# hits-mbm-dev/grappa

Measured on AMD Instinct MI355X. Metric: molecules/sec (train step, energy+force loss), higher is better.
Workload: dtype f32

## Files before the change

### grappa_amd/_lib.py

```python
import ctypes as C
import os

_HERE = os.path.dirname(os.path.abspath(__file__))
LIB_PATH = os.environ.get("GRAPPA_HIP_LIB") or os.path.join(_HERE, "libgrappa_hip.so")

ABI_VERSION = 11
GEMM_GROUP4_MAX = 4
GEMM_GROUP_MAX = 16
GEMM_PRECISIONS = {"f32": 0, "f32_bf16x9": 1, "f32_bf16x6": 2, "bf16x3": 3, "bf16": 4, "f32_f16x3": 5}

c_float_p = C.POINTER(C.c_float)
c_int_p = C.POINTER(C.c_int)


class GemmDesc(C.Structure):
    _fields_ = [("M", C.c_int), ("N", C.c_int), ("K", C.c_int), ("a_kcontig", C.c_int), ("b_kcontig", C.c_int),
                ("A", C.c_void_p), ("lda", C.c_int), ("B", C.c_void_p), ("ldb", C.c_int), ("C", C.c_void_p), ("ldc", C.c_int),
                ("C2", C.c_void_p), ("ldc2", C.c_int), ("bias", C.c_void_p), ("res", C.c_void_p), ("ldres", C.c_int),
                ("aux", C.c_void_p), ("ldaux", C.c_int), ("pre", C.c_void_p), ("ldpre", C.c_int), ("a_colsum", C.c_void_p), ("act", C.c_int), ("drop_p", C.c_float), ("drop_seed", C.c_uint64),
                ("accumulate", C.c_int), ("precision", C.c_int),
                ("a_planes", C.c_int), ("b_planes", C.c_int), ("a_plane_stride", C.c_size_t), ("b_plane_stride", C.c_size_t),
                ("Cp", C.c_void_p), ("ldcp", C.c_int), ("cp_plane_stride", C.c_size_t),
                ("resp", C.c_void_p), ("ldresp", C.c_int), ("resp_plane_stride", C.c_size_t),
                ("auxp", C.c_void_p), ("ldauxp", C.c_int), ("auxp_plane_stride", C.c_size_t),
# ... 74 lines not shown
                ("n1_gamma", C.c_void_p), ("n1_beta", C.c_void_p), ("nf_gamma", C.c_void_p), ("nf_beta", C.c_void_p),
                ("drop_p", C.c_float), ("seed1", C.c_uint64), ("seed2", C.c_uint64), ("drop_salt", C.c_void_p),
                ("save_mean1", C.c_void_p), ("save_rstd1", C.c_void_p), ("save_meanf", C.c_void_p), ("save_rstdf", C.c_void_p),
                ("save_x1", C.c_void_p), ("save_qkv", C.c_void_p), ("save_att", C.c_void_p), ("save_x2", C.c_void_p), ("save_x3", C.c_void_p),
                ("save_u", C.c_void_p), ("gather_idx", C.c_void_p), ("x1_tab", C.c_void_p), ("qkv_tab", C.c_void_p), ("x2_tiled", C.c_int)]


class WriterLayerBwdDesc(C.Structure):
    _fields_ = [("s", C.c_int), ("T", C.c_int), ("F", C.c_int), ("nheads", C.c_int), ("dtype", C.c_int), ("dout", C.c_void_p),
                ("x", C.c_void_p), ("qkv", C.c_void_p), ("x2", C.c_void_p), ("u", C.c_void_p),
                ("mean1", C.c_void_p), ("rstd1", C.c_void_p), ("meanf", C.c_void_p), ("rstdf", C.c_void_p),
                ("n1_gamma", C.c_void_p), ("nf_gamma", C.c_void_p),
                ("w_in_tpk", C.c_void_p), ("w_o_tpk", C.c_void_p), ("w1_tpk", C.c_void_p), ("w2_tpk", C.c_void_p),
                ("drop_p", C.c_float), ("seed1", C.c_uint64), ("seed2", C.c_uint64), ("drop_salt", C.c_void_p),
                ("dx", C.c_void_p), ("dz2", C.c_void_p), ("dz1", C.c_void_p), ("dzo", C.c_void_p), ("dqkv", C.c_void_p),
                ("ln1_part", C.c_void_p), ("lnf_part", C.c_void_p), ("x2_tiled", C.c_int), ("gather_idx", C.c_void_p)]


WRITER_BF16 = 1

EVAL_NMOM = 10
EVAL_METRICS = ("std_energies", "std_gradients", "rmse_energies", "mae_energies", "rmse_gradients", "crmse_gradients", "mae_gradients")

COLLATE_MODES = {"copy": 0, "add": 1, "inv_rows": 2, "inc_code": 3, "conf": 4}

VP4 = C.c_void_p * 4
VP6 = C.c_void_p * 6

_vp, _i, _f, _sz, _u64 = C.c_void_p, C.c_int, C.c_float, C.c_size_t, C.c_uint64
SIGNATURES = {
    "grappa_abi_version": (_i, []),
    "grappa_build_arch": (C.c_char_p, []),
    "grappa_launch_count": (C.c_longlong, [_i]),
    "grappa_adam_step_dyn_f32": (_i, [_vp, _sz, _vp, _vp, _vp, _vp, _vp, _f, _f, _f, _f, _vp, _f, _vp, _f]),
    "grappa_split_planes_f32": (_i, [_vp, _i, _i, _vp, _i, _vp, _i, _sz, _i]),
    "grappa_split_pairs_f32": (_i, [_vp, _i, _i, _vp, _i, _vp, _vp, _i, _i]),
    "grappa_split_pairs_f32_batched": (_i, [_vp, _i, _i, _vp]),
    "grappa_amax_f32_workspace_bytes": (_sz, [_i, _i]),
    "grappa_amax_f32": (_i, [_vp, _i, _i, _vp, _i, _vp, _vp, _vp, _sz]),
    "grappa_amax_f32_batched": (_i, [_vp, _i, _vp]),
    "grappa_amax_reduce": (_i, [_vp, _i, C.POINTER(C.c_void_p), C.POINTER(C.c_int), _vp]),
    "grappa_amax_combine": (_i, [_vp, _i, _i, _vp, _vp]),
    "grappa_gemm_f32_workspace_bytes": (_sz, [_i, _i, _i]),
    "grappa_gemm_f32_plan": (_i, [_i, _i, _i, _i, c_int_p, c_int_p, c_int_p, c_int_p, c_int_p]),
    "grappa_gemm_f32_plan_desc": (_i, [C.POINTER(GemmDesc), c_int_p, c_int_p, c_int_p, c_int_p, c_int_p]),
    "grappa_gemm_f32_workspace_bytes_desc": (_sz, [C.POINTER(GemmDesc)]),
    "grappa_gemm_f32": (_i, [_vp, C.POINTER(GemmDesc), _vp, _sz]),
    "grappa_gemm_f32_grouped_workspace_bytes": (_sz, [C.POINTER(GemmDesc), _i]),
    "grappa_gemm_f32_grouped": (_i, [_vp, C.POINTER(GemmDesc), _i, _vp, _sz]),
    "grappa_gemm_f32_group_workspace_bytes": (_sz, [C.POINTER(GemmDesc), _i]),
    "grappa_gemm_f32_group": (_i, [_vp, C.POINTER(GemmDesc), _i, _vp, _sz]),
    "grappa_colsum_workspace_bytes": (_sz, [_i, _i]),
    "grappa_colsum_f32": (_i, [_vp, _i, _i, _vp, _i, _vp, _i, _vp, _sz]),
    "grappa_act_dropout_bwd_f32": (_i, [_vp, _i, _i, _vp, _i, _vp, _i, _f, _u64, _vp, _i, _vp]),
    "grappa_act_dropout_bwd_amax_f32": (_i, [_vp, _i, _i, _vp, _i, _vp, _i, _f, _u64, _vp, _i, _vp, _vp]),
    "grappa_layernorm_fwd_batched_f32": (_i, [_vp, C.POINTER(LnFwdItem), _i]),
    "grappa_layernorm_bwd_batched_f32": (_i, [_vp, C.POINTER(LnBwdItem), _i]),
    "grappa_act_dropout_bwd_batched_f32": (_i, [_vp, C.POINTER(ActDropoutItem), _i]),
    "grappa_seqattn_fwd_batched_f32": (_i, [_vp, C.POINTER(SeqAttnItem), _i]),
    "grappa_seqattn_bwd_batched_f32": (_i, [_vp, C.POINTER(SeqAttnItem), _i]),
    "grappa_act_dropout_bwd_pairs_f32": (_i, [_vp, _i, _i, _vp, _i, _vp, _i, _f, _u64, _vp, _i, _vp, _vp, _i, _vp]),
    "grappa_add_f32": (_i, [_vp, _sz, _vp, _vp, _vp]),
    "grappa_layernorm_fwd_f32": (_i, [_vp, _i, _i, _vp, _i, _vp, _vp, _vp, _i, _vp, _vp]),
    "grappa_layernorm_fwd_pairs_f32": (_i, [_vp, _i, _i, _vp, _i, _vp, _vp, _vp, _i, _vp, _vp, _vp, _vp, _i]),
    "grappa_layernorm_fwd_amax_f32": (_i, [_vp, _i, _i, _vp, _i, _vp, _vp, _vp, _i, _vp, _vp, _vp]),
    "grappa_layernorm_bwd_workspace_bytes": (_sz, [_i, _i]),
    "grappa_layernorm_bwd_partial_rows": (_i, [_i]),
    "grappa_colsum_partials_batched": (_i, [_vp, C.POINTER(ColsumItem), _i]),
    "grappa_layernorm_bwd_f32": (_i, [_vp, _i, _i, _vp, _i, _vp, _i, _vp, _vp, _vp, _vp, _i, _vp, _vp, _i, _vp, _sz]),
    "grappa_layernorm_bwd_amax_f32": (_i, [_vp, _i, _i, _vp, _i, _vp, _i, _vp, _vp, _vp, _vp, _i, _vp, _vp, _i, _vp, _sz, _vp]),
    "grappa_layernorm_bwd_drop_f32": (_i, [_vp, _i, _i, _vp, _i, _vp, _i, _vp, _vp, _vp, _vp, _i, _vp, _vp, _i, _vp, _sz, _vp, _f, _u64, _vp, _i, _vp, _vp]),
    "grappa_gat_fwd_f32": (_i, [_vp, _i, _i, _i, _i, _vp, _vp, _vp, _vp, _vp]),
    "grappa_gat_bwd_f32": (_i, [_vp, _i, _i, _i, _i, _vp, _vp, _vp, _vp, _vp, _vp, _vp, _vp, _vp]),
    "grappa_neighbor_mean_f32": (_i, [_vp, _i, _i, _vp, _vp, _vp, _vp, _i]),
    "grappa_neighbor_mean_bf16": (_i, [_vp, _i, _i, _vp, _vp, _vp, _vp, _i, _i]),
    "grappa_charge_encoding_f32": (_i, [_vp, _i, _vp, _i, _f, _f, _vp, _i, _i]),
    "grappa_tuple_gather_fwd_f32": (_i, [_vp, _i, _i, _i, _vp, _i, _vp, _vp, _vp, _i]),
    "grappa_tuple_gather_bwd_f32": (_i, [_vp, _i, _i, _vp, _vp, _vp, _i, _vp, _i, _i, _i]),
    "grappa_seqattn_fwd_f32": (_i, [_vp, _i, _i, _i, _i, _vp, _vp]),
    "grappa_seqattn_fwd_pairs_f32": (_i, [_vp, _i, _i, _i, _i, _vp, _vp, _i, _vp]),
    "grappa_seqattn_bwd_f32": (_i, [_vp, _i, _i, _i, _i, _vp, _vp, _vp]),
    "grappa_seqattn_fwd_amax_f32": (_i, [_vp, _i, _i, _i, _i, _vp, _vp, _vp]),
    "grappa_seqattn_bwd_amax_f32": (_i, [_vp, _i, _i, _i, _i, _vp, _vp, _vp, _vp]),
    "grappa_perm_concat_fwd_f32": (_i, [_vp, _i, _i, _i, _i, c_int_p, _vp, _vp]),
    "grappa_perm_concat_bwd_f32": (_i, [_vp, _i, _i, _i, _i, c_int_p, _vp, _vp]),
    "grappa_param_out_fwd_f32": (_i, [_vp, _i, _i, _i, _i, _i, _f, _vp, _i, _vp, _vp, _vp]),
    "grappa_param_out_bwd_f32": (_i, [_vp, _i, _i, _i, _i, _i, _f, _vp, _i, _vp, _vp, _vp, _vp]),
    "grappa_param_out_stats_workspace_bytes": (_sz, [_i]),
    "grappa_param_out_bwd_stats_f32": (_i, [_vp, _i, _i, _i, _i, _i, _f, _vp, _i, _vp, _vp, _vp, _vp, _vp, _sz]),
    "grappa_mm_energy_fwd_f32": (_i, [_vp, C.POINTER(MMDesc), _vp, _vp, C.POINTER(VP4), C.POINTER(VP4)]),
    "grappa_mm_gradient_fwd_f32": (_i, [_vp, C.POINTER(MMDesc), _vp]),
    "grappa_mm_bwd_f32": (_i, [_vp, C.POINTER(MMDesc), _vp, _vp, C.POINTER(VP4), C.POINTER(VP4)]),
    "grappa_nonbonded_iblock": (_i, []),
    "grappa_nonbonded_workspace_bytes": (_sz, [_i, _i, _i]),
    "grappa_nonbonded_fwd_f32": (_i, [_vp, C.POINTER(NbDesc), _vp, _vp, _vp, _vp, _sz]),
    "grappa_nonbonded_plan": (C.c_longlong, [_i, _i, _i, _vp, _vp, C.c_longlong]),
    "grappa_nonbonded_fwd_planned_f32": (_i, [_vp, C.POINTER(NbDesc), _vp, _i, _i, _vp, _vp, _vp, _vp, _sz]),
    "grappa_relax_max_atoms": (_i, []),
    "grappa_relax_fire_f32": (_i, [_vp, C.POINTER(MMDesc), C.POINTER(NbDesc), C.POINTER(RelaxOpts), _vp, _vp, _vp, _vp, _vp, _vp, _vp]),
    "grappa_relax_steps_workspace_bytes": (_sz, [_i, _i, _i, _i]),
    "grappa_relax_steps_init_f32": (_i, [_vp, C.POINTER(MMDesc), C.POINTER(NbDesc), C.POINTER(RelaxOpts), _vp, _i, _i, _vp, _sz, _vp]),
    "grappa_relax_steps_run_f32": (_i, [_vp, C.POINTER(MMDesc), C.POINTER(NbDesc), C.POINTER(RelaxOpts), _vp, _i, _i, _vp, _sz, _i, _vp]),
    "grappa_relax_steps_finish_f32": (_i, [_vp, C.POINTER(MMDesc), C.POINTER(NbDesc), C.POINTER(RelaxOpts), _vp, _i, _i, _vp, _sz,
                                           _vp, _vp, _vp, _vp, _vp, _vp, _vp]),
    "grappa_md_langevin_f32": (_i, [_vp, C.POINTER(MMDesc), C.POINTER(NbDesc), C.POINTER(MdOpts), _vp, _vp, _vp, _vp, _vp, _vp, _vp, _vp, _vp,
                                    _vp, _vp, _vp]),
    "grappa_md_philox": (None, [_u64, C.c_uint, C.c_uint, C.c_uint, C.c_uint, C.POINTER(C.c_uint * 4)]),
    "grappa_md_noise_f32": (_i, [_vp, _vp, _vp, _i, _i, _i, C.c_uint, C.c_uint, _vp]),
    "grappa_loss_ef_fwd_bwd_f32": (_i, [_vp, _i, _i, _i, _vp, _vp, _vp, _vp, _vp, _vp, _f, _f, _f, _vp, _vp, _vp]),
    "grappa_loss_param_fwd_bwd_f32": (_i, [_vp, C.POINTER(PLossDesc), _vp, C.POINTER(VP6)]),
    "grappa_eval_se_f32": (_i, [_vp, _i, _i, _i, _vp, _vp, _vp, _vp, _vp, _vp, _vp]),
    "grappa_eval_moments_f32": (_i, [_vp, _i, _i, _i, _vp, _vp, _vp, _vp, _vp, _vp, _vp]),
    "grappa_eval_bootstrap_f64": (_i, [_vp, _vp, _i, _i, _vp, _vp, _i, _i, _i, _vp, _vp, _vp]),
    "grappa_collate_batch": (_i, [_vp, _vp, C.POINTER(CollateDesc), _i, _i]),
    "grappa_sumsq_workspace_bytes": (_sz, [_sz]),
    "grappa_sumsq_f32": (_i, [_vp, _sz, _vp, _vp, _i, _vp, _sz]),
    "grappa_adam_step_f32": (_i, [_vp, _sz, _vp, _vp, _vp, _vp, _f, _f, _f, _f, _f, _i, _f, _vp, _f]),
    "grappa_dropout_keep": (_i, [_u64, _u64, _f]),
    "grappa_layernorm_fwd_bf16": (_i, [_vp, _i, _i, _vp, _i, _vp, _vp, _vp, _i, _vp, _vp]),
    "grappa_layernorm_bwd_bf16": (_i, [_vp, _i, _i, _vp, _i, _vp, _i, _vp, _vp, _vp, _vp, _i, _vp, _vp, _i, _vp, _sz]),
    "grappa_act_dropout_bwd_bf16": (_i, [_vp, _i, _i, _vp, _i, _vp, _i, _f, _u64, _vp, _i, _vp]),
    "grappa_gat_fwd_bf16": (_i, [_vp, _i, _i, _i, _i, _vp, _vp, _vp, _vp, _vp]),
    "grappa_gat_bwd_bf16": (_i, [_vp, _i, _i, _i, _i, _vp, _vp, _vp, _vp, _vp, _vp, _vp, _vp, _vp]),
    "grappa_tuple_gather_fwd_bf16": (_i, [_vp, _i, _i, _i, _vp, _i, _vp, _vp, _vp, _i]),
    "grappa_tuple_gather_bwd_bf16": (_i, [_vp, _i, _i, _vp, _vp, _vp, _i, _vp, _i, _i, _i]),
    "grappa_seqattn_fwd_bf16": (_i, [_vp, _i, _i, _i, _i, _vp, _vp]),
    "grappa_seqattn_bwd_bf16": (_i, [_vp, _i, _i, _i, _i, _vp, _vp, _vp]),
    "grappa_perm_concat_fwd_bf16": (_i, [_vp, _i, _i, _i, _i, c_int_p, _vp, _vp]),
    "grappa_perm_concat_bwd_bf16": (_i, [_vp, _i, _i, _i, _i, c_int_p, _vp, _vp]),
    "grappa_convert_f32_to_bf16": (_i, [_vp, _i, _i, _vp, _i, _vp, _i]),
    "grappa_convert_bf16_to_f32": (_i, [_vp, _i, _i, _vp, _i, _vp, _i]),
    "grappa_writer_head_fwd": (_i, [_vp, C.POINTER(WriterLayerDesc)]),
    "grappa_writer_head_bwd": (_i, [_vp, C.POINTER(WriterLayerBwdDesc)]),
    "grappa_writer_head_tiles": (_i, [_i, _i]),
    "grappa_writer_pack_bytes": (_sz, [_i, _i, _i]),
    "grappa_writer_pack_weight": (_i, [_vp, _i, _i, _vp, _i, _i, _i, _vp]),
}

_lib = None


def load():
    global _lib
    if _lib is not None:
        return _lib
    if not os.path.exists(LIB_PATH):
        raise RuntimeError(f"{LIB_PATH} is missing: build it with `python -c 'import __graft_entry__ as g; g.build()'` "
                           f"or `make -C grappa_amd/csrc` (there is no CPU fallback for the Grappa HIP path)")
    lib = C.CDLL(LIB_PATH)
    for name, (res, args) in SIGNATURES.items():
        fn = getattr(lib, name)
        fn.restype = res
        fn.argtypes = args
    if lib.grappa_abi_version() != ABI_VERSION:
        raise RuntimeError("libgrappa_hip.so: ABI version mismatch")
    _lib = lib
    return lib


def nonbonded_iblock() -> int:
    return int(load().grappa_nonbonded_iblock())


def relax_max_atoms() -> int:
    return int(load().grappa_relax_max_atoms())

# ... 6 lines not shown
```

### grappa_amd/backend.py

```python
from __future__ import annotations

import ctypes as C
import os
import weakref
from collections import namedtuple
from typing import List, NamedTuple, Optional, Sequence

import torch

from . import _lib
from ._marshal import GrappaHipError, _chk, _flat, _ptr
from .backend_mm import MMBackend

_BACKEND = None


def set_backend(b) -> None:
    global _BACKEND
    _BACKEND = b


def get_backend():
    global _BACKEND
    if _BACKEND is None:
# ... 64 lines not shown
    precision: int

    @property
    def fmt(self) -> str:
        return self.name if self.name in ("pairs", "wpairs") else ("planes" if self.name.endswith("planes") else "f32")

    @property
    def fp16_split(self) -> bool:
        return self.name in ("pairs", "wpairs", "split")


class _PendingGemm:
    __slots__ = ("d", "route", "shape", "flops", "nbytes", "ret", "dev", "keep", "groupable", "key")

    def __init__(self, d, route, shape, flops, nbytes, ret, dev, keep, groupable):
        self.d, self.route, self.shape, self.flops, self.nbytes, self.ret, self.dev, self.keep, self.groupable = d, route, shape, flops, nbytes, ret, dev, keep, groupable
        self.key = (route.name, route.name == "split" and route.layout, route.precision)


_PlanesEntry = namedtuple("_PlanesEntry", "ver planes ref")
_PairsTable = namedtuple("_PairsTable", "tab n tiles keep")
_AmaxTable = namedtuple("_AmaxTable", "tab n")
_PairsRefresh = namedtuple("_PairsRefresh", "event captured ordered")
_WgradItem = namedtuple("_WgradItem", "dz x dw db am pz px")
_LnItem = namedtuple("_LnItem", "part nrows W dgamma_ptr dbeta_ptr dgamma dbeta stream task")


class _PairsEntry:
    __slots__ = ("ver", "pairs", "ref", "epoch", "transposed", "amax")

    def __init__(self, ver, pairs, ref, epoch, transposed, amax):
        self.ver, self.pairs, self.ref, self.epoch, self.transposed, self.amax = ver, pairs, ref, epoch, transposed, amax


class _AmaxEntry:
    __slots__ = ("ver", "w", "amax", "epoch", "batchable")

    def __init__(self, ver, w, amax, epoch, batchable):
        self.ver, self.w, self.amax, self.epoch, self.batchable = ver, w, amax, epoch, batchable


class HipBackend(MMBackend):
    name = "hip"

    def __init__(self):
        if not torch.cuda.is_available():
            raise RuntimeError("grappa_amd needs an AMD GPU (torch.cuda.is_available() is False); there is no CPU fallback")
        self.lib = _lib.load()
        self._ws = {}
        self._ws_need = {}
        self.set_gemm_precision(os.environ.get("GRAPPA_GEMM_PRECISION", DEFAULT_GEMM_PRECISION))
        self.set_gemm_precision_bwd(os.environ.get("GRAPPA_GEMM_PRECISION_BWD") or None)
        self._prof = None
        self.defer_wgrads = os.environ.get("GRAPPA_DEFER_WGRADS", "1") not in ("0", "")
        self._wq = {}
        self.defer_ln = os.environ.get("GRAPPA_DEFER_LN_REDUCTIONS", "1") not in ("0", "")
        self._lnq = []
        self._tasks = set()
        self.wgrad_queue_bytes = int(float(os.environ.get("GRAPPA_WGRAD_QUEUE_GB", "12")) * 2 ** 30)
        self.inference_pairs = os.environ.get("GRAPPA_INFERENCE_PAIRS", "1") not in ("0", "")
        self.training_pairs = os.environ.get("GRAPPA_TRAINING_PAIRS", "1") not in ("0", "")
        self.group_launches = os.environ.get("GRAPPA_GROUP_LAUNCHES", "1") not in ("0", "")
        self.amax_parts = os.environ.get("GRAPPA_AMAX_PARTS", "0") not in ("0", "")
        self.fuse_ln_drop = os.environ.get("GRAPPA_FUSE_LN_DROP", "1") not in ("0", "")
        self.pairs_min_rows = int(os.environ.get("GRAPPA_PAIRS_MIN_ROWS", "12288"))
        self.backward_pairs = os.environ.get("GRAPPA_BACKWARD_PAIRS", "0") not in ("0", "")
        self.weight_pairs_min_rows = int(os.environ.get("GRAPPA_WPAIRS_MIN_ROWS", "24000"))
        self._tails = None
        self._salt = None
        self._salt_ptr = None
        self.plan_override = None
        self.splitk_reduce = 0
        self._tails_pinned = False
        if os.environ.get("GRAPPA_PLAN_TAILS", "") != "":
            self.pin_tail_launches(os.environ["GRAPPA_PLAN_TAILS"] != "0")
        self.gnn_tails = os.environ.get("GRAPPA_GNN_TAILS", "0") not in ("0", "")
        self.wgrads_aside = os.environ.get("GRAPPA_WGRADS_ASIDE", "1") not in ("0", "")
        self._side_streams = {}
        self._aside = []
        self.weight_planes = os.environ.get("GRAPPA_WEIGHT_PLANES", "0") not in ("0", "")
        self.fused_writer_layer = os.environ.get("GRAPPA_FUSED_WRITER_LAYER", "1") not in ("0", "")
        self.fused_writer_layer_bwd = os.environ.get("GRAPPA_FUSED_WRITER_LAYER_BWD", "1") not in ("0", "")
        self.fused_first_layer = os.environ.get("GRAPPA_FUSED_FIRST_LAYER", "1") not in ("0", "")
        self._wplanes = {}
        self._wpairs = {}
        self._wptable = None
        self._wpairs_ready = None
        self._wepoch = 0
        self._wamax = {}
        self._wtable = None
        self.wgrad_column_maxima = os.environ.get("GRAPPA_WGRAD_COLUMN_MAXIMA", "0") not in ("0", "")

    def set_gemm_precision(self, name: str) -> None:
        if name not in _lib.GEMM_PRECISIONS:
            raise ValueError(f"gemm precision {name!r}: expected one of {sorted(_lib.GEMM_PRECISIONS)}")
        self.gemm_precision_name = name
        self.gemm_precision = _lib.GEMM_PRECISIONS[name]

    def set_gemm_precision_bwd(self, name) -> None:
        if name is not None and name not in _lib.GEMM_PRECISIONS:
            raise ValueError(f"gemm precision {name!r}: expected one of {sorted(_lib.GEMM_PRECISIONS)}")
        self.gemm_precision_bwd_name = name
        self.gemm_precision_bwd = None if name is None else _lib.GEMM_PRECISIONS[name]

    def invalidate_weight_planes(self) -> None:
        self._wepoch += 1

    def invalidate_weights(self) -> None:
        self._wepoch += 1

    def _cached_form(self, w: torch.Tensor, tag, alloc, fill) -> torch.Tensor:
        key = (w.data_ptr(), *w.shape, tag)
        ver = (w._version, self._wepoch)
        hit = self._wplanes.get(key)
        if hit is not None and hit.ref() is not w:
            hit = None
        if hit is not None and hit.ver == ver:
            return hit.planes
        if hit is not None:
            t = hit.planes
        else:
            t = alloc()
            for k in [k for k, e in self._wplanes.items() if e.ref() is None]:
                del self._wplanes[k]
        fill(t)
        self._wplanes[key] = _PlanesEntry(ver, t, weakref.ref(w))
        return t

    def _planes_of_weight(self, w: torch.Tensor, transposed: bool) -> torch.Tensor:
        R, Cc = w.shape
        rows, cols = (Cc, R) if transposed else (R, Cc)
        return self._cached_form(
            w, transposed, lambda: torch.zeros((3, (rows + 31) // 32 * 32, (cols + 31) // 32 * 32), dtype=torch.bfloat16, device=w.device),
            lambda pl: _chk(self.lib.grappa_split_planes_f32(self._stream(), R, Cc, w.data_ptr(), _f32_2d(w, "W", w.device), pl.data_ptr(), pl.stride(1),
                                                             pl.stride(0), int(transposed)), "grappa_split_planes_f32"))

    def _pairs_of_weight(self, w: torch.Tensor, transposed: bool = False) -> torch.Tensor:
        R, Cc = w.shape
        key = (w.data_ptr(), R, Cc, "pairsT" if transposed else "pairs")
        ver = (w._version, self._wepoch)
        hit = self._wpairs.get(key)
        if hit is not None and hit.ref() is not w:
            hit = None
        if hit is not None:
            hit.epoch = self._wepoch
            if hit.ver == ver:
                self._after_pairs_refresh()
                return hit.pairs
            self._refresh_weight_pairs()
            if hit.ver == ver:
                return hit.pairs
        am = self._amax_of_weight(w)
        rows, cols = (Cc, R) if transposed else (R, Cc)
        pairs = torch.zeros((rows, 2 * ((cols + 31) // 32 * 32)), dtype=torch.float16, device=w.device)
        _chk(self.lib.grappa_split_pairs_f32(self._stream(), R, Cc, w.data_ptr(), _f32_2d(w, "W", w.device), (am.col if transposed else am.row).data_ptr(),
                                             pairs.data_ptr(), pairs.stride(0), int(transposed)), "grappa_split_pairs_f32")
        for k in [k for k, e in self._wpairs.items() if e.ref() is None]:
            del self._wpairs[k]
        self._wpairs[key] = _PairsEntry(ver, pairs, weakref.ref(w), self._wepoch, transposed, am)
        self._wptable = None
        return pairs

    def _refresh_weight_pairs(self) -> None:
        import numpy as np
        ageing = not torch.cuda.is_current_stream_capturing()
        for k in [k for k, e in self._wpairs.items() if e.ref() is None or (ageing and e.epoch < self._wepoch - 1)]:
# ... 958 lines not shown
    def _csr_check(self, plan, N, dev):
        if plan.N != N or plan.indptr.device != dev or plan.indptr.dtype != torch.int32 or plan.indptr.numel() != N + 1:
            raise ValueError("graph plan does not match the feature tensor (atoms / device)")
        if plan.indices.numel() != plan.E or plan.rev.numel() != plan.E:
            raise ValueError("graph plan: edge arrays")

    def gat_fwd(self, plan, ft, H, D, out, alpha) -> None:
        dev = out.device
        N = ft.shape[0]
        self._csr_check(plan, N, dev)
        dt = _same_dtype(ft, out)
        _flat(ft, "ft", dev, dt), _flat(out, "out", dev, dt), _flat(alpha, "alpha", dev)
        if ft.shape[1] != H * D or out.shape != ft.shape or alpha.numel() != plan.E * H:
            raise ValueError("gat_fwd: shapes")
        eb = ft.element_size()
        nbytes = plan.E * (H * D * eb + 4) + N * (2 * H * D * eb + 4)
        fn = getattr(self.lib, f"grappa_gat_fwd_{_sfx(ft)}")
        self._timed("gat_fwd", 2.0 * plan.E * H * D * 2, nbytes,
                    lambda: _chk(fn(self._stream(), N, plan.E, H, D, plan.indptr.data_ptr(), plan.indices.data_ptr(),
                                    ft.data_ptr(), out.data_ptr(), alpha.data_ptr()), "grappa_gat_fwd"))

    def gat_bwd(self, plan, ft, out, alpha, dout, H, D, dft) -> None:
        dev = dft.device
        N = ft.shape[0]
        self._csr_check(plan, N, dev)
        dt = _same_dtype(ft, out, dout, dft)
        for t, n in ((ft, "ft"), (out, "out"), (dout, "dout"), (dft, "dft")):
            _flat(t, n, dev, dt)
        _flat(alpha, "alpha", dev)
        if ft.shape[1] != H * D or out.shape != ft.shape or dout.shape != ft.shape or dft.shape != ft.shape or alpha.numel() != plan.E * H:
            raise ValueError("gat_bwd: shapes")
        delta = torch.empty((N, H), dtype=torch.float32, device=dev)
        eb = ft.element_size()
        nbytes = plan.E * (2 * H * D * eb + 4) + N * (4 * H * D * eb + 4)
        fn = getattr(self.lib, f"grappa_gat_bwd_{_sfx(ft)}")
        self._timed("gat_bwd", 2.0 * plan.E * H * D * 5, nbytes,
                    lambda: _chk(fn(self._stream(), N, plan.E, H, D, plan.indptr.data_ptr(), plan.indices.data_ptr(),
                                    plan.rev.data_ptr(), ft.data_ptr(), out.data_ptr(), alpha.data_ptr(), dout.data_ptr(),
                                    dft.data_ptr(), delta.data_ptr()), "grappa_gat_bwd"))

    def neighbor_mean(self, plan, x, out, scale_by_neighbor: bool) -> None:
        dev = out.device
        N, F = x.shape
        self._csr_check(plan, N, dev)
        if out.shape != x.shape:
            raise ValueError("neighbor_mean: shapes")
        if x.dtype == torch.bfloat16:
            _flat(x, "x", dev, torch.bfloat16), _flat(out, "out", dev, out.dtype)
            if out.dtype not in _ACT_DTYPES:
                raise ValueError("neighbor_mean: out must be bfloat16 or float32")
            _chk(self.lib.grappa_neighbor_mean_bf16(self._stream(), N, F, plan.indptr.data_ptr(), plan.indices.data_ptr(), x.data_ptr(), out.data_ptr(),
                                                    int(out.dtype == torch.float32), int(scale_by_neighbor)), "grappa_neighbor_mean_bf16")
            return
        _flat(x, "x", dev), _flat(out, "out", dev)
        _chk(self.lib.grappa_neighbor_mean_f32(self._stream(), N, F, plan.indptr.data_ptr(), plan.indices.data_ptr(), x.data_ptr(), out.data_ptr(),
                                               int(scale_by_neighbor)), "grappa_neighbor_mean_f32")

    def charge_encoding(self, q, dim, lo, hi, out, col0) -> None:
        dev = out.device
        _flat(q, "q", dev)
        N = q.numel()
        if out.shape[0] != N or col0 + dim > out.shape[1]:
            raise ValueError("charge_encoding: shapes")
        _chk(self.lib.grappa_charge_encoding_f32(self._stream(), N, q.data_ptr(), dim, float(lo), float(hi), out.data_ptr(), _f32_2d(out, "out", dev),
                                                 col0), "grappa_charge_encoding_f32")

    def tuple_gather_fwd(self, a, idx, s, pe, x) -> None:
        dev = x.device
        T = idx.shape[0]
        W = x.shape[1]
        if idx.dtype != torch.int32 or idx.device != dev or not idx.is_contiguous() or (T and idx.shape[1] != s):
            raise ValueError("tuple_gather_fwd: idx must be contiguous int32 (T,s)")
        if x.shape[0] != s * T or a.shape[1] < W:
            raise ValueError("tuple_gather_fwd: shapes")
        if pe is not None:
            _flat(pe, "pe", dev)
            if pe.numel() != s:
                raise ValueError("tuple_gather_fwd: pe length")
        dt = _same_dtype(a, x)
        fn = getattr(self.lib, f"grappa_tuple_gather_fwd_{_sfx(x)}")
        _chk(fn(self._stream(), T, s, W, a.data_ptr(), _f32_2d(a, "a", dev, dt), idx.data_ptr(), _ptr(pe),
                x.data_ptr(), _f32_2d(x, "x", dev, dt)), "grappa_tuple_gather_fwd")

    def tuple_gather_bwd(self, inv_ptr, inv_rows, dx, da, has_pe: bool, accumulate=False) -> None:
        dev = da.device
        N, W = da.shape[0], dx.shape[1]
        if inv_ptr.dtype != torch.int32 or inv_ptr.numel() != N + 1 or inv_ptr.device != dev or inv_rows.dtype != torch.int32:
            raise ValueError("tuple_gather_bwd: inverse incidence")
        if da.shape[1] < W or inv_rows.numel() != dx.shape[0]:
            raise ValueError("tuple_gather_bwd: shapes")
        dt = _same_dtype(dx, da)
        fn = getattr(self.lib, f"grappa_tuple_gather_bwd_{_sfx(da)}")
        _chk(fn(self._stream(), N, W, inv_ptr.data_ptr(), inv_rows.data_ptr(), dx.data_ptr(),
                _f32_2d(dx, "dx", dev, dt), da.data_ptr(), _f32_2d(da, "da", dev, dt), int(has_pe), int(accumulate)),
             "grappa_tuple_gather_bwd")

    def seqattn_fwd(self, qkv, s, T, nheads, out, amax=None, pairs=False):
        if pairs:
            dev = qkv.device
            F = qkv.shape[1] // 3
            if qkv.dtype != torch.float32 or qkv.shape != (s * T, 3 * F) or F % nheads or F % 32 or F > 512:
                raise ValueError("seqattn_fwd: the pair format needs float32 q, k, v of F % 32 == 0, F <= 512 columns each")
            _flat(qkv, "qkv", dev)
            row = torch.empty(s * T, dtype=torch.int32, device=dev)
            pr = torch.empty((s * T, 2 * F), dtype=torch.float16, device=dev)
            if T:
                _chk(self.lib.grappa_seqattn_fwd_pairs_f32(self._stream(), s, T, nheads, F // nheads, qkv.data_ptr(), pr.data_ptr(), pr.stride(0),
                                                           row.data_ptr()), "grappa_seqattn_fwd_pairs_f32")
            return Amax(row=row, pairs=pr)
        dev = out.device
        dt = _same_dtype(qkv, out)
        _flat(qkv, "qkv", dev, dt), _flat(out, "out", dev, dt)
        F = out.shape[1]
        if qkv.shape != (s * T, 3 * F) or out.shape[0] != s * T or F % nheads:
            raise ValueError("seqattn_fwd: shapes")
        row = self._new_row_amax(out, False, amax)
        args = (self._stream(), s, T, nheads, F // nheads, qkv.data_ptr(), out.data_ptr())
        if row is not None:
            _chk(self.lib.grappa_seqattn_fwd_amax_f32(*args, row.data_ptr()), "grappa_seqattn_fwd_amax_f32")
            return Amax(row=row)
        _chk(getattr(self.lib, f"grappa_seqattn_fwd_{_sfx(out)}")(*args), "grappa_seqattn_fwd")
        return None

    def _packed_weight(self, w: torch.Tensor, transposed: bool = False) -> torch.Tensor:
        R, Cc = w.shape
        N, K = (Cc, R) if transposed else (R, Cc)
        return self._cached_form(
            w, "packT" if transposed else "pack", lambda: torch.empty(N * K, dtype=torch.bfloat16, device=w.device),
            lambda pk: _chk(self.lib.grappa_writer_pack_weight(self._stream(), N, K, w.data_ptr(), _f32_2d(w, "W", w.device), int(transposed), _lib.WRITER_BF16,
                                                               pk.data_ptr()), "grappa_writer_pack_weight"))

    def writer_layer_ok(self, x: torch.Tensor, s: int, nheads: int, *params) -> bool:
        if not self.fused_writer_layer or x.dtype != torch.bfloat16 or x.dim() != 2 or x.shape[1] != 512 or nheads != 8 or s not in (2, 3, 4):
            return False
        if x.shape[0] == 0:
            return False
        return all(p is not None and p.dtype == torch.float32 and p.is_contiguous() for p in params)

    def writer_layer_fwd(self, x, s, T, nheads, drop_p, seed1, seed2, n1_w, n1_b, w_in, b_in, w_o, b_o, nf_w, nf_b, w1, b1, w2, b2, out, save=None, gather=None):
        dev = out.device
        M, Fd = out.shape
        d = _lib.WriterLayerDesc()
        d.s, d.T, d.F, d.nheads, d.dtype = s, T, Fd, nheads, _lib.WRITER_BF16
        _flat(out, "out", dev, torch.bfloat16)
        d.out = out.data_ptr()
        if gather is not None:
            idx_tab, x1_tab, qkv_tab = gather
            if M != s * T or idx_tab.dtype != torch.int32 or tuple(idx_tab.shape) != (T, s) or not idx_tab.is_contiguous() or idx_tab.device != dev:
                raise ValueError("writer_layer_fwd: gather index")
            _flat(x1_tab, "x1_tab", dev, torch.bfloat16), _flat(qkv_tab, "qkv_tab", dev, torch.bfloat16)
            if x1_tab.shape[1] != Fd or tuple(qkv_tab.shape) != (x1_tab.shape[0], 3 * Fd):
                raise ValueError("writer_layer_fwd: gather tables")
            d.gather_idx, d.x1_tab, d.qkv_tab = idx_tab.data_ptr(), x1_tab.data_ptr(), qkv_tab.data_ptr()
        else:
            if tuple(x.shape) != (M, Fd) or M != s * T or out.dtype != x.dtype:
                raise ValueError("writer_layer_fwd: shapes")
            _flat(x, "x", dev, torch.bfloat16)
            d.x = x.data_ptr()
        for name, wt, shape in (("w_in_pk", w_in, (3 * Fd, Fd)), ("w_o_pk", w_o, (Fd, Fd)), ("w1_pk", w1, (Fd, Fd)), ("w2_pk", w2, (Fd, Fd))):
            if gather is not None and name == "w_in_pk":
                continue
            if tuple(wt.shape) != shape:
                raise ValueError(f"writer_layer_fwd: {name[:-3]} has shape {tuple(wt.shape)}, expected {shape}")
            setattr(d, name, self._packed_weight(wt).data_ptr())
        for name, v, n in (("b_in", b_in, 3 * Fd), ("b_o", b_o, Fd), ("b1", b1, Fd), ("b2", b2, Fd), ("n1_gamma", n1_w, Fd), ("n1_beta", n1_b, Fd),
                           ("nf_gamma", nf_w, Fd), ("nf_beta", nf_b, Fd)):
            if gather is not None and name.startswith("n1_"):
                continue
            _flat(v, name, dev)
            if v.numel() != n:
                raise ValueError(f"writer_layer_fwd: {name} length")
            setattr(d, name, v.data_ptr())
        d.drop_p, d.seed1, d.seed2 = float(drop_p), int(seed1) & (2 ** 64 - 1), int(seed2) & (2 ** 64 - 1)
        d.drop_salt = self._salt_ptr
        keep = None
        if save is not None:
            for name in ("meanf", "rstdf") if gather is not None else ("mean1", "rstd1", "meanf", "rstdf"):
                t = save[name]
                _flat(t, name, dev)
                if t.numel() != M:
                    raise ValueError(f"writer_layer_fwd: save[{name!r}] length")
                setattr(d, "save_" + name, t.data_ptr())
            tiles = self.lib.grappa_writer_head_tiles(s, T)
            d.x2_tiled = int(bool(save.get("x2_tiled", False)))
            for name in ("att", "x2", "x3", "u") if gather is not None else ("x1", "qkv", "att", "x2", "x3", "u"):
                t = save[name]
                _flat(t, name, dev, torch.bfloat16)
                want = (tiles * 64, Fd) if (name == "x2" and d.x2_tiled) else (M, 3 * Fd if name == "qkv" else Fd)
                if tuple(t.shape) != want:
                    raise ValueError(f"writer_layer_fwd: save[{name!r}] shape {tuple(t.shape)}, expected {want}")
                setattr(d, "save_" + name, t.data_ptr())
            keep = save
        nprod = 3 if gather is not None else 6
        flops = 2.0 * M * Fd * (nprod * Fd) + 4.0 * M * s * Fd
        nbytes = 2.0 * M * Fd * ((5 if gather is not None else 2) + ((5 if gather is not None else 9) if save is not None else 0)) + 2.0 * nprod * Fd * Fd
        self._timed("writer_layer", flops, nbytes, lambda: _chk(self.lib.grappa_writer_head_fwd(self._stream(), C.byref(d)), "grappa_writer_head_fwd"),
                    lambda: [{"M": M, "s": s, "save": keep is not None, "gather": gather is not None}])

    def writer_layer_bwd(self, dout, x, s, T, nheads, drop_p, seed1, seed2, saved, n1_w, n1_b, w_in, w_o, nf_w, nf_b, w1, w2, gather=None):
        dev = dout.device
        M, Fd = dout.shape
        bf = torch.bfloat16
        if M != s * T:
            raise ValueError("writer_layer_bwd: shapes")
        d = _lib.WriterLayerBwdDesc()
        d.s, d.T, d.F, d.nheads, d.dtype = s, T, Fd, nheads, _lib.WRITER_BF16
        ntiles = self.lib.grappa_writer_head_tiles(s, T)
        d.x2_tiled = int(bool(saved.get("x2_tiled", False)))
        if gather is not None:
            idx_tab, qkv_tab = gather
            if idx_tab.dtype != torch.int32 or tuple(idx_tab.shape) != (T, s) or not idx_tab.is_contiguous() or qkv_tab.shape[1] != 3 * Fd:
                raise ValueError("writer_layer_bwd: gather arguments")
            d.gather_idx = idx_tab.data_ptr()
            tensors = (("dout", dout, (M, Fd)), ("qkv", qkv_tab, tuple(qkv_tab.shape)), ("x2", saved["x2"], (ntiles * 64, Fd) if d.x2_tiled else (M, Fd)),
                       ("u", saved["u"], (M, Fd)))
        else:
            tensors = (("dout", dout, (M, Fd)), ("x", x, (M, Fd)), ("qkv", saved["qkv"], (M, 3 * Fd)),
                       ("x2", saved["x2"], (ntiles * 64, Fd) if d.x2_tiled else (M, Fd)), ("u", saved["u"], (M, Fd)))
        for name, t, shape in tensors:
            _flat(t, name, dev, bf)
            if tuple(t.shape) != shape:
                raise ValueError(f"writer_layer_bwd: {name} shape")
            setattr(d, name, t.data_ptr())
        for name in ("meanf", "rstdf") if gather is not None else ("mean1", "rstd1", "meanf", "rstdf"):
            _flat(saved[name], name, dev)
            setattr(d, name, saved[name].data_ptr())
        _flat(nf_w, "nf_gamma", dev)
        d.nf_gamma = nf_w.data_ptr()
        if gather is None:
            _flat(n1_w, "n1_gamma", dev)
            d.n1_gamma = n1_w.data_ptr()
        for name, wt in (("w_in_tpk", w_in), ("w_o_tpk", w_o), ("w1_tpk", w1), ("w2_tpk", w2)):
            if gather is not None and name == "w_in_tpk":
                continue
            setattr(d, name, self._packed_weight(wt, transposed=True).data_ptr())
        d.drop_p, d.seed1, d.seed2, d.drop_salt = float(drop_p), int(seed1) & (2 ** 64 - 1), int(seed2) & (2 ** 64 - 1), self._salt_ptr
        new = lambda *sh: torch.empty(sh, dtype=bf, device=dev)
        dx, dz2, dz1, dzo, dqkv = new(M, Fd), new(M, Fd), new(M, Fd), new(M, Fd), new(M, 3 * Fd)
        parts = torch.empty((2, ntiles, 2, Fd), dtype=torch.float32, device=dev)
        d.dx, d.dz2, d.dz1, d.dzo, d.dqkv = dx.data_ptr(), dz2.data_ptr(), dz1.data_ptr(), dzo.data_ptr(), dqkv.data_ptr()
        d.ln1_part, d.lnf_part = parts[0].data_ptr(), parts[1].data_ptr()
        nprod = 3 if gather is not None else 6
        flops = 2.0 * M * Fd * (nprod * Fd) + 8.0 * M * s * Fd
        self._timed("writer_layer", flops, 2.0 * M * Fd * 15 + 2.0 * nprod * Fd * Fd,
                    lambda: _chk(self.lib.grappa_writer_head_bwd(self._stream(), C.byref(d)), "grappa_writer_head_bwd"),
                    lambda: [{"M": M, "s": s, "bwd": True, "gather": gather is not None}])
        for part, g, b in ((parts[1], nf_w, nf_b),) if gather is not None else ((parts[0], n1_w, n1_b), (parts[1], nf_w, nf_b)):
            self._reduce_ln_partials(part, ntiles, Fd, g, b)
        return dx, dz2, dz1, dzo, dqkv

    def _reduce_ln_partials(self, part, nrows, W, gamma, beta) -> None:
        from .ops import _pgrad
        dg = _pgrad(gamma) if gamma.requires_grad else torch.zeros_like(gamma)
        db = _pgrad(beta) if beta.requires_grad else torch.zeros_like(beta)
        task = self._queue_flush() if (self.defer_wgrads and self.defer_ln) else -1
        if task >= 0 and all(q.dgamma_ptr != dg.data_ptr() for q in self._lnq if q.task == task):
            self._lnq.append(_LnItem(part, nrows, W, dg.data_ptr(), db.data_ptr(), dg, db, torch.cuda.current_stream(), task))
            return
        arr = (_lib.ColsumItem * 1)()
        a = arr[0]
        a.part, a.nrows, a.n, a.out, a.out2, a.n_first, a.accumulate = part.data_ptr(), nrows, 2 * W, dg.data_ptr(), db.data_ptr(), W, 1
        _chk(self.lib.grappa_colsum_partials_batched(self._stream(), arr, 1), "grappa_colsum_partials_batched")

    def seqattn_bwd(self, qkv, dout, s, T, nheads, dqkv, amax=None):
        dev = dqkv.device
        dt = _same_dtype(qkv, dout, dqkv)
        _flat(qkv, "qkv", dev, dt), _flat(dout, "dout", dev, dt), _flat(dqkv, "dqkv", dev, dt)
        F = dout.shape[1]
        if qkv.shape != (s * T, 3 * F) or dqkv.shape != qkv.shape or dout.shape[0] != s * T:
            raise ValueError("seqattn_bwd: shapes")
        row = self._new_row_amax(dqkv, True, amax)
        args = (self._stream(), s, T, nheads, F // nheads, qkv.data_ptr(), dout.data_ptr(), dqkv.data_ptr())
        if row is not None:
            _chk(self.lib.grappa_seqattn_bwd_amax_f32(*args, row.data_ptr()), "grappa_seqattn_bwd_amax_f32")
            return Amax(row=row)
        _chk(getattr(self.lib, f"grappa_seqattn_bwd_{_sfx(dqkv)}")(*args), "grappa_seqattn_bwd")
        return None

    def perm_concat_fwd(self, x, s, T, perms: Sequence[Sequence[int]], z) -> None:
        dev = z.device
        dt = _same_dtype(x, z)
        _flat(x, "x", dev, dt), _flat(z, "z", dev, dt)
        F, P = x.shape[1], len(perms)
        if x.shape[0] != s * T or z.shape != (P * T, s * F):
            raise ValueError("perm_concat_fwd: shapes")
        arr = (C.c_int * (P * s))(*[int(v) for p in perms for v in p])
        fn = getattr(self.lib, f"grappa_perm_concat_fwd_{_sfx(z)}")
        _chk(fn(self._stream(), s, T, F, P, arr, x.data_ptr(), z.data_ptr()), "grappa_perm_concat_fwd")

    def perm_concat_bwd(self, dz, s, T, perms, dx) -> None:
        dev = dx.device
        dt = _same_dtype(dz, dx)
        _flat(dz, "dz", dev, dt), _flat(dx, "dx", dev, dt)
        F, P = dx.shape[1], len(perms)
        if dx.shape[0] != s * T or dz.shape != (P * T, s * F):
            raise ValueError("perm_concat_bwd: shapes")
        arr = (C.c_int * (P * s))(*[int(v) for p in perms for v in p])
        fn = getattr(self.lib, f"grappa_perm_concat_bwd_{_sfx(dx)}")
        _chk(fn(self._stream(), s, T, F, P, arr, dz.data_ptr(), dx.data_ptr()), "grappa_perm_concat_bwd")

    def param_out_fwd(self, kind, o, T, P, n_per, gated, cutoff, consts, k, eq) -> None:
        dev = k.device
        _flat(o, "o", dev), _flat(consts, "consts", dev), _flat(k, "k", dev)
        if o.shape[0] != P * T:
            raise ValueError("param_out_fwd: shapes")
        if eq is not None:
            _flat(eq, "eq", dev)
        _chk(self.lib.grappa_param_out_fwd_f32(self._stream(), kind, T, P, n_per, int(gated), float(cutoff), o.data_ptr(), o.shape[1],
                                               consts.data_ptr(), k.data_ptr(), _ptr(eq)), "grappa_param_out_fwd_f32")

    def param_out_bwd(self, kind, o, T, P, n_per, gated, cutoff, consts, dk, deq, d_o) -> None:
        dev = d_o.device
        _flat(o, "o", dev), _flat(consts, "consts", dev), _flat(d_o, "d_o", dev)
        for t, n in ((dk, "dk"), (deq, "deq")):
            if t is not None:
                _flat(t, n, dev)
        if o.shape[0] != P * T or d_o.shape != o.shape:
            raise ValueError("param_out_bwd: shapes")
        _chk(self.lib.grappa_param_out_bwd_f32(self._stream(), kind, T, P, n_per, int(gated), float(cutoff), o.data_ptr(), o.shape[1],
                                               consts.data_ptr(), _ptr(dk), _ptr(deq), d_o.data_ptr()), "grappa_param_out_bwd_f32")

    def param_out_bwd_stats(self, kind, o, T, P, n_per, gated, cutoff, consts, dk, deq, d_consts) -> None:
        dev = d_consts.device
        _flat(o, "o", dev), _flat(consts, "consts", dev), _flat(d_consts, "d_consts", dev)
        if o.shape[0] != P * T or d_consts.numel() != consts.numel():
            raise ValueError("param_out_bwd_stats: shapes")
        ws = self._workspace(self.lib.grappa_param_out_stats_workspace_bytes(T), dev)
        _chk(self.lib.grappa_param_out_bwd_stats_f32(self._stream(), kind, T, P, n_per, int(gated), float(cutoff), _ptr(o), o.shape[1] if o.dim() == 2 else 0,
                                                     consts.data_ptr(), _ptr(dk), _ptr(deq), d_consts.data_ptr(), ws.data_ptr(), ws.numel()),
             "grappa_param_out_bwd_stats_f32")

    def loss_ef(self, plan, energy, energy_ref, is_dummy, grad, grad_ref, wE, wG, inv_B, loss_mol, gE, gG) -> None:
        dev = loss_mol.device
        B = _loss_mols(plan)
        Cc = energy.shape[1] if energy is not None else grad.shape[1]
        for t, n in ((energy, "energy"), (energy_ref, "energy_ref"), (is_dummy, "is_dummy"), (grad, "grad"), (grad_ref, "grad_ref"),
                     (gE, "gE"), (gG, "gG"), (loss_mol, "loss_mol")):
            if t is not None:
                _flat(t, n, dev)
        _chk(self.lib.grappa_loss_ef_fwd_bwd_f32(self._stream(), B, Cc, plan.N, plan.atom_molptr.data_ptr(), _ptr(energy), _ptr(energy_ref),
                                                 _ptr(is_dummy), _ptr(grad), _ptr(grad_ref), float(wE), float(wG), float(inv_B),
                                                 loss_mol.data_ptr(), _ptr(gE), _ptr(gG)), "grappa_loss_ef_fwd_bwd_f32")

    def collate_gather(self, tables, B: int) -> None:
        if not tables or B == 0:
            return
        dev = tables[0]["dst"].device
        arr = (_lib.CollateDesc * len(tables))()
        for d, t in zip(arr, tables):
            for k in ("src", "dst"):
                if t[k].element_size() not in (4, 8) or t[k].device != dev or not t[k].is_contiguous():
                    raise ValueError(f"collate table {k}: expected a contiguous 4- or 8-byte tensor on {dev}")
            for k, dt in (("src_row", torch.int64), ("dst_row", torch.int64), ("p0", torch.int32), ("p1", torch.int32)):
                v = t.get(k)
# ... 130 lines not shown
```

### grappa_amd/capture.py

```python
from __future__ import annotations

from typing import Callable, Dict, Optional, Tuple

import torch

from .backend import get_backend


def _pinned_by_graph(be):
    return (list(be._wamax.values()), be._wtable, list(be._wpairs.values()), be._wptable, dict(be._wplanes), dict(be._ws), getattr(be, "_salt", None),
            dict(be._side_streams))


def _touch_weight_caches(be) -> None:
    for e in be._wamax.values():
        e.epoch = be._wepoch
    for e in be._wpairs.values():
        e.epoch = be._wepoch


def _drop_outputs(g) -> None:
    for lvl in ("n2", "n3", "n4", "n4_improper"):
        for k in ("k", "eq"):
            g.nodes[lvl].data.pop(k, None)
# ... 186 lines not shown
        self.plan = g.plan()
        for lvl in ("n2", "n3", "n4", "n4_improper"):
            if self.plan.T[lvl]:
                self.plan.position_tables(lvl)
        self.signature = train_signature(g)
        self._rehome_inputs()
        self.stream = torch.cuda.Stream(device=g.device)
        self.stream.wait_stream(torch.cuda.current_stream(g.device))
        with torch.cuda.stream(self.stream), torch.no_grad():
            for _ in range(max(int(warmup), 3)):
                self.be.invalidate_weights()
                self._eager()
        self.stream.synchronize()
        self.be.invalidate_weights()
        self.graph = torch.cuda.CUDAGraph()
        with torch.cuda.graph(self.graph, stream=self.stream), torch.no_grad():
            self._eager()
        self._pinned = _pinned_by_graph(self.be)
        torch.cuda.current_stream(g.device).wait_stream(self.stream)

    def _eager(self):
        _drop_outputs(self.g)
        return self.energy(self.model(self.g))

    def __call__(self):
        self.graph.replay()
        _touch_weight_caches(self.be)
        return self.g


def train_signature(g) -> tuple:
    plan = g.plan()
    return (tuple(int(g.num_nodes(nt)) for nt in ("n1", "n2", "n3", "n4", "n4_improper", "g")), int(g.num_edges()), getattr(plan, "n_real_mols", None),
            tuple(sorted((nt, k, tuple(v.shape), str(v.dtype)) for nt, d in g._data.items() for k, v in d.items() if torch.is_tensor(v))))


class CapturedForward:

    def __init__(self, model, g, warmup: int = 2, refresh_weights: bool = False):
        self.model, self.g = model, g
        self.refresh_weights = bool(refresh_weights)
        self.be = get_backend()
        self.plan = g.plan()
        for lvl in ("n2", "n3", "n4", "n4_improper"):
            if self.plan.T[lvl]:
                self.plan.position_tables(lvl)
        self._rehome_inputs()
        self.stream = torch.cuda.Stream(device=g.device)
        self.stream.wait_stream(torch.cuda.current_stream(g.device))
        with torch.cuda.stream(self.stream), torch.no_grad():
            for _ in range(max(int(warmup), 3 if self.refresh_weights else 1)):
                if self.refresh_weights:
                    self.be.invalidate_weights()
                _drop_outputs(g)
                model(g)
        self.stream.synchronize()
        if self.refresh_weights:
            self.be.invalidate_weights()
        self.weights_stamp = self._stamp()
        self.config_stamp = self._config_stamp()
        self.graph = torch.cuda.CUDAGraph()
        with torch.cuda.graph(self.graph, stream=self.stream), torch.no_grad():
            _drop_outputs(g)
            model(g)
            self.outputs: Dict[Tuple[str, str], torch.Tensor] = {(lvl, k): g.nodes[lvl].data[k] for lvl in ("n2", "n3", "n4", "n4_improper")
                                                                for k in ("k", "eq") if k in g.nodes[lvl].data}
            self.out_flat = torch.cat([t.reshape(-1).float() for t in self.outputs.values()]) if self.outputs else None
        self._pinned = _pinned_by_graph(self.be)
        torch.cuda.current_stream(g.device).wait_stream(self.stream)
        self.out_host = torch.empty(self.out_flat.shape, dtype=torch.float32).pin_memory() if self.out_flat is not None else None

    def _stamp(self):
        ps = self.__dict__.get("_params")
        if ps is None:
            ps = self._params = list(self.model.parameters())
        return (self.be._wepoch, sum(p._version for p in ps))

    def _config_stamp(self):
        be = self.be
        ps = self.__dict__.get("_params")
        if ps is None:
            ps = self._params = list(self.model.parameters())
        return (be.gemm_precision_name, getattr(be, "gemm_precision_bwd", None), be.inference_pairs, be.training_pairs, be._tails, be.plan_override,
                be.splitk_reduce, be.weight_pairs_min_rows, be.pairs_min_rows, tuple(p.data_ptr() for p in ps))

    def valid(self) -> bool:
        if self._config_stamp() != self.config_stamp:
            return False
        return self.refresh_weights or self._stamp() == self.weights_stamp

    def replay(self):
        self.graph.replay()
        if self.refresh_weights:
            _touch_weight_caches(self.be)
        return self.g

    @staticmethod
    def signature(g) -> tuple:
        return (tuple(int(g.num_nodes(nt)) for nt in ("n1", "n2", "n3", "n4", "n4_improper", "g")), int(g.num_edges()),
                tuple(sorted((k, tuple(v.shape), str(v.dtype)) for k, v in g._data["n1"].items() if torch.is_tensor(v) and k != "h")))

    @staticmethod
    def _plan_tensors(plan):
        out = {}
        for name, val in vars(plan).items():
            if torch.is_tensor(val):
                out[name] = val
            elif isinstance(val, dict):
                for k, v in val.items():
                    if torch.is_tensor(v):
                        out[f"{name}.{k}"] = v
                    elif isinstance(v, tuple):
                        for i, t in enumerate(v):
                            if torch.is_tensor(t):
                                out[f"{name}.{k}.{i}"] = t
        return out

    def _input_slots(self, plan, g):
        slots = dict(self._plan_tensors(plan))
        for k, t in g._data["n1"].items():
            if torch.is_tensor(t) and k != "h":
                slots["n1." + k] = t
        return slots

    def _rehome_inputs(self) -> None:
        slots = self._input_slots(self.plan, self.g)
        self._layout, off = {}, 0
        for name, t in slots.items():
            nbytes = t.numel() * t.element_size()
            self._layout[name] = (off, nbytes, t.dtype, tuple(t.shape))
            off += (nbytes + 15) // 16 * 16
        self._in_dev = torch.zeros(max(off, 16), dtype=torch.uint8, device=self.g.device)
        self._in_host = torch.zeros(max(off, 16), dtype=torch.uint8).pin_memory()
        self._host_views = {name: self._in_host[o:o + nbytes].view(dtype).view(shape) for name, (o, nbytes, dtype, shape) in self._layout.items()}
        views = {}
        for name, (o, nbytes, dtype, shape) in self._layout.items():
            v = self._in_dev[o:o + nbytes].view(dtype).view(shape)
            v.copy_(slots[name])
            views[name] = v
        for name, v in views.items():
            parts = name.split(".")
            if parts[0] == "n1":
                self.g._data["n1"][name[3:]] = v
            elif len(parts) == 1:
                setattr(self.plan, name, v)
            elif len(parts) == 2:
                getattr(self.plan, parts[0])[parts[1]] = v
            else:
                d = getattr(self.plan, parts[0])
                tup = list(d[parts[1]])
                tup[int(parts[2])] = v
                d[parts[1]] = tuple(tup)

    def load(self, g_host) -> None:
        plan = g_host.plan()
        for lvl in self.plan.__dict__.get("_pos_tables", {}):
            plan.position_tables(lvl)
        src = self._input_slots(plan, g_host)
        if set(src) != set(self._layout):
            raise ValueError("load: the graph has other input tables than the captured one")
        for name, (o, nbytes, dtype, shape) in self._layout.items():
            t = src[name]
            if tuple(t.shape) != shape or t.dtype != dtype:
                raise ValueError(f"load: {name} is {t.dtype} {tuple(t.shape)}, the captured graph holds {dtype} {shape}")
            self._host_views[name].copy_(t)
        self._in_dev.copy_(self._in_host, non_blocking=True)

# ... 49 lines not shown
```

### grappa_amd/csrc/tuples.hip

```cpp
#include "common.h"

namespace {

struct Perms {
    int p[6][4];
};

template <typename TA, typename TX>
__global__ __launch_bounds__(256) void tuple_gather_fwd_kernel(int T, int s, int W, const TA* __restrict__ a, int lda,
                                                               const int* __restrict__ idx, const float* __restrict__ pe,
                                                               TX* __restrict__ x, int ldx) {
    const int lane = threadIdx.x & 63;
    const int nrows = s * T, nvec = W >> 2;
    const int wave0 = (blockIdx.x * blockDim.x + threadIdx.x) >> 6, nw = (gridDim.x * blockDim.x) >> 6;
    for (int r = wave0; r < nrows; r += nw) {
        const int pos = r / T, t = r - pos * T;
        const int atom = idx[(size_t)t * s + pos];
        const TA* src = a + (size_t)atom * lda;
        TX* dst = x + (size_t)r * ldx;
        const float pev = pe ? pe[pos] : 0.f;
        for (int c = lane; c < nvec; c += 64) {
            float4 v = ld4(src, c);
            if (pe && c == nvec - 1) v.w = pev;
            st4(dst, c, v);
        }
    }
}

template <typename TX, typename TA>
__global__ __launch_bounds__(256) void tuple_gather_bwd_kernel(int N, int W, const int* __restrict__ inv_ptr, const int* __restrict__ inv_rows,
                                                               const TX* __restrict__ dx, int lddx, TA* __restrict__ da, int ldda,
                                                               int has_pe, int accumulate) {
    const int lane = threadIdx.x & 63;
    const int nvec = W >> 2;
    const int n = (blockIdx.x * blockDim.x + threadIdx.x) >> 6;
    if (n >= N) return;
    const int r0 = inv_ptr[n], r1 = inv_ptr[n + 1];
    TA* dst = da + (size_t)n * ldda;
    for (int c = lane; c < nvec; c += 64) {
        float4 acc = accumulate ? ld4(dst, c) : make_float4(0.f, 0.f, 0.f, 0.f);
        for (int j = r0; j < r1; ++j) {
            float4 v = ld4(dx + (size_t)inv_rows[j] * lddx, c);
            if (has_pe && c == nvec - 1) v.w = 0.f;
            acc.x += v.x; acc.y += v.y; acc.z += v.z; acc.w += v.w;
        }
        st4(dst, c, acc);
    }
}

__device__ inline float dot4(const float4& a, const float4& b) { return (a.x * b.x + a.y * b.y) + (a.z * b.z + a.w * b.w); }

__device__ inline unsigned mag4(const float4& v) {
    return max(max(__float_as_uint(v.x) & 0x7fffffffu, __float_as_uint(v.y) & 0x7fffffffu),
               max(__float_as_uint(v.z) & 0x7fffffffu, __float_as_uint(v.w) & 0x7fffffffu));
}
__device__ inline unsigned wave_umax(unsigned v) {
#pragma unroll
    for (int o = 32; o > 0; o >>= 1) v = max(v, (unsigned)__shfl_xor((int)v, o, 64));
    return v;
}

template <int S, typename TE>
__device__ __forceinline__ void seqattn_fwd_body(int T, int F, int dh, const TE* __restrict__ qkv, TE* __restrict__ out,
                                                 unsigned* __restrict__ row_amax, int vblock) {
    const int lane = threadIdx.x & 63;
    const int t = (vblock * blockDim.x + threadIdx.x) >> 6;
    if (t >= T) return;
    const int nvec = F >> 2, lph = dh >> 2;
    const float scale = 1.0f / sqrtf((float)dh);
    unsigned am[S];
#pragma unroll
    for (int i = 0; i < S; ++i) am[i] = 0u;
    for (int c0 = 0; c0 < nvec; c0 += 64) {
        const int c = c0 + lane;
        const bool ok = c < nvec;
        float4 q[S], k[S], v[S];
#pragma unroll
        for (int i = 0; i < S; ++i) {
            const TE* row = qkv + ((size_t)i * T + t) * 3 * F;
            q[i] = ok ? ld4(row, c) : make_float4(0.f, 0.f, 0.f, 0.f);
            k[i] = ok ? ld4(row, nvec + c) : make_float4(0.f, 0.f, 0.f, 0.f);
            v[i] = ok ? ld4(row, 2 * nvec + c) : make_float4(0.f, 0.f, 0.f, 0.f);
        }
#pragma unroll
        for (int i = 0; i < S; ++i) {
            float sc[S], mx = -INFINITY;
#pragma unroll
            for (int j = 0; j < S; ++j) {
                sc[j] = group_sum(dot4(q[i], k[j]), lph) * scale;
                mx = fmaxf(mx, sc[j]);
            }
            float den = 0.f;
#pragma unroll
            for (int j = 0; j < S; ++j) {
                sc[j] = expf(sc[j] - mx);
                den += sc[j];
            }
            const float inv = 1.0f / den;
            float4 o = make_float4(0.f, 0.f, 0.f, 0.f);
#pragma unroll
            for (int j = 0; j < S; ++j) {
                const float p = sc[j] * inv;
                o.x += p * v[j].x; o.y += p * v[j].y; o.z += p * v[j].z; o.w += p * v[j].w;
            }
            if (ok) {
                st4(out + ((size_t)i * T + t) * F, c, o);
                am[i] = max(am[i], mag4(o));
            }
        }
    }
    if (row_amax) {
#pragma unroll
        for (int i = 0; i < S; ++i) {
            const unsigned m = wave_umax(am[i]);
            if (lane == 0) row_amax[(size_t)i * T + t] = m;
        }
    }
}

template <int S, typename TE>
__global__ __launch_bounds__(256) void seqattn_fwd_kernel(int T, int F, int dh, const TE* __restrict__ qkv, TE* __restrict__ out,
                                                          unsigned* __restrict__ row_amax) {
    seqattn_fwd_body<S, TE>(T, F, dh, qkv, out, row_amax, blockIdx.x);
}

struct SeqAttnBatch {
    grappa_seqattn_item it[GRAPPA_ROW_BATCH_MAX];
    int blk_begin[GRAPPA_ROW_BATCH_MAX + 1];
    int count;
};
__global__ __launch_bounds__(256) void seqattn_fwd_batched_kernel(SeqAttnBatch b) {
    int i = 0;
    while (i + 1 < b.count && (int)blockIdx.x >= b.blk_begin[i + 1]) ++i;
    const grappa_seqattn_item& t = b.it[i];
    const int vb = (int)blockIdx.x - b.blk_begin[i], F = t.nheads * t.dh;
    switch (t.s) {
        case 1: seqattn_fwd_body<1, float>(t.T, F, t.dh, t.qkv, t.out, t.amax, vb); break;
        case 2: seqattn_fwd_body<2, float>(t.T, F, t.dh, t.qkv, t.out, t.amax, vb); break;
        case 3: seqattn_fwd_body<3, float>(t.T, F, t.dh, t.qkv, t.out, t.amax, vb); break;
        default: seqattn_fwd_body<4, float>(t.T, F, t.dh, t.qkv, t.out, t.amax, vb); break;
    }
}

template <int S>
__global__ __launch_bounds__(256) void seqattn_fwd_pairs_kernel(int T, int F, int dh, const float* __restrict__ qkv, uint16_t* __restrict__ pairs, int ldp,
                                                                unsigned* __restrict__ row_amax) {
    const int lane = threadIdx.x & 63;
    const int t = (blockIdx.x * blockDim.x + threadIdx.x) >> 6;
    if (t >= T) return;
    const int nvec = F >> 2, lph = dh >> 2;
    const float scale = 1.0f / sqrtf((float)dh);
    unsigned am[S];
    float4 keep[2][S];
#pragma unroll
    for (int i = 0; i < S; ++i) am[i] = 0u;
#pragma unroll
    for (int trip = 0; trip < 2; ++trip) {
        const int c = trip * 64 + lane;
        const bool ok = c < nvec;
        float4 q[S], k[S], v[S];
#pragma unroll
        for (int i = 0; i < S; ++i) {
            const float* row = qkv + ((size_t)i * T + t) * 3 * F;
            q[i] = ok ? ld4(row, c) : make_float4(0.f, 0.f, 0.f, 0.f);
            k[i] = ok ? ld4(row, nvec + c) : make_float4(0.f, 0.f, 0.f, 0.f);
            v[i] = ok ? ld4(row, 2 * nvec + c) : make_float4(0.f, 0.f, 0.f, 0.f);
        }
#pragma unroll
        for (int i = 0; i < S; ++i) {
            float sc[S], mx = -INFINITY;
#pragma unroll
            for (int j = 0; j < S; ++j) {
                sc[j] = group_sum(dot4(q[i], k[j]), lph) * scale;
                mx = fmaxf(mx, sc[j]);
            }
            float den = 0.f;
#pragma unroll
            for (int j = 0; j < S; ++j) {
                sc[j] = expf(sc[j] - mx);
                den += sc[j];
            }
            const float inv = 1.0f / den;
            float4 o = make_float4(0.f, 0.f, 0.f, 0.f);
#pragma unroll
            for (int j = 0; j < S; ++j) {
                const float p = sc[j] * inv;
                o.x += p * v[j].x; o.y += p * v[j].y; o.z += p * v[j].z; o.w += p * v[j].w;
            }
            keep[trip][i] = o;
            if (ok) am[i] = max(am[i], mag4(o));
        }
    }
#pragma unroll
    for (int i = 0; i < S; ++i) {
        const unsigned m = wave_umax(am[i]);
        const int shift = grappa_amax_shift(m);
        uint16_t* pr = pairs + ((size_t)i * T + t) * ldp;
#pragma unroll
        for (int trip = 0; trip < 2; ++trip) {
            const int c = trip * 64 + lane;
            st_pairs4_paired(pr, c, keep[trip][i], shift, c < nvec);
        }
        if (lane == 0) row_amax[(size_t)i * T + t] = m;
    }
}

template <int S, typename TE>
__device__ __forceinline__ void seqattn_bwd_body(int T, int F, int dh, const TE* __restrict__ qkv, const TE* __restrict__ dout,
                                                 TE* __restrict__ dqkv, unsigned* __restrict__ row_amax, int vblock) {
    const int lane = threadIdx.x & 63;
    const int t = (vblock * blockDim.x + threadIdx.x) >> 6;
    if (t >= T) return;
    const int nvec = F >> 2, lph = dh >> 2;
    const float scale = 1.0f / sqrtf((float)dh);
    const float4 zero = make_float4(0.f, 0.f, 0.f, 0.f);
    unsigned am[S];
#pragma unroll
    for (int i = 0; i < S; ++i) am[i] = 0u;
    for (int c0 = 0; c0 < nvec; c0 += 64) {
        const int c = c0 + lane;
        const bool ok = c < nvec;
        float4 q[S], k[S], v[S], go[S], dq[S], dk[S], dv[S];
#pragma unroll
        for (int i = 0; i < S; ++i) {
            const TE* row = qkv + ((size_t)i * T + t) * 3 * F;
            q[i] = ok ? ld4(row, c) : zero;
            k[i] = ok ? ld4(row, nvec + c) : zero;
            v[i] = ok ? ld4(row, 2 * nvec + c) : zero;
            go[i] = ok ? ld4(dout + ((size_t)i * T + t) * F, c) : zero;
            dq[i] = zero; dk[i] = zero; dv[i] = zero;
        }
#pragma unroll
        for (int i = 0; i < S; ++i) {
            float p[S], dp[S], mx = -INFINITY;
#pragma unroll
            for (int j = 0; j < S; ++j) {
                p[j] = group_sum(dot4(q[i], k[j]), lph) * scale;
                mx = fmaxf(mx, p[j]);
            }
            float den = 0.f;
#pragma unroll
            for (int j = 0; j < S; ++j) {
                p[j] = expf(p[j] - mx);
                den += p[j];
            }
            const float inv = 1.0f / den;
            float dsum = 0.f;
#pragma unroll
            for (int j = 0; j < S; ++j) {
                p[j] *= inv;
                dp[j] = group_sum(dot4(go[i], v[j]), lph);
                dsum += p[j] * dp[j];
            }
#pragma unroll
            for (int j = 0; j < S; ++j) {
                const float ds = p[j] * (dp[j] - dsum) * scale;
                dq[i].x += ds * k[j].x; dq[i].y += ds * k[j].y; dq[i].z += ds * k[j].z; dq[i].w += ds * k[j].w;
                dk[j].x += ds * q[i].x; dk[j].y += ds * q[i].y; dk[j].z += ds * q[i].z; dk[j].w += ds * q[i].w;
                dv[j].x += p[j] * go[i].x; dv[j].y += p[j] * go[i].y; dv[j].z += p[j] * go[i].z; dv[j].w += p[j] * go[i].w;
            }
        }
        if (ok) {
#pragma unroll
            for (int i = 0; i < S; ++i) {
                TE* row = dqkv + ((size_t)i * T + t) * 3 * F;
                st4(row, c, dq[i]);
                st4(row, nvec + c, dk[i]);
                st4(row, 2 * nvec + c, dv[i]);
                am[i] = max(am[i], max(mag4(dq[i]), max(mag4(dk[i]), mag4(dv[i]))));
            }
        }
    }
    if (row_amax) {
#pragma unroll
        for (int i = 0; i < S; ++i) {
            const unsigned m = wave_umax(am[i]);
            if (lane == 0) row_amax[(size_t)i * T + t] = m;
        }
    }
}

template <int S, typename TE>
__global__ __launch_bounds__(256) void seqattn_bwd_kernel(int T, int F, int dh, const TE* __restrict__ qkv, const TE* __restrict__ dout,
                                                          TE* __restrict__ dqkv, unsigned* __restrict__ row_amax) {
    seqattn_bwd_body<S, TE>(T, F, dh, qkv, dout, dqkv, row_amax, blockIdx.x);
}

__global__ __launch_bounds__(256) void seqattn_bwd_batched_kernel(SeqAttnBatch b) {
    int i = 0;
    while (i + 1 < b.count && (int)blockIdx.x >= b.blk_begin[i + 1]) ++i;
    const grappa_seqattn_item& t = b.it[i];
    const int vb = (int)blockIdx.x - b.blk_begin[i], F = t.nheads * t.dh;
    switch (t.s) {
        case 1: seqattn_bwd_body<1, float>(t.T, F, t.dh, t.qkv, t.dout, t.dqkv, t.amax, vb); break;
        case 2: seqattn_bwd_body<2, float>(t.T, F, t.dh, t.qkv, t.dout, t.dqkv, t.amax, vb); break;
        case 3: seqattn_bwd_body<3, float>(t.T, F, t.dh, t.qkv, t.dout, t.dqkv, t.amax, vb); break;
        default: seqattn_bwd_body<4, float>(t.T, F, t.dh, t.qkv, t.dout, t.dqkv, t.amax, vb); break;
    }
}

template <int S, int E, typename TE>
__global__ __launch_bounds__(256) void seqattn_fwd_kernel_e(int T, int F, int dh, const TE* __restrict__ qkv, TE* __restrict__ out) {
    const int lane = threadIdx.x & 63;
    const int t = (blockIdx.x * blockDim.x + threadIdx.x) >> 6;
    if (t >= T) return;
    const int nvec = F / E, lph = dh / E;
    const float scale = 1.0f / sqrtf((float)dh);
    for (int c0 = 0; c0 < nvec; c0 += 64) {
        const int c = c0 + lane;
        const bool ok = c < nvec;
        Chunk<E> q[S], k[S], v[S];
#pragma unroll
        for (int i = 0; i < S; ++i) {
            const TE* row = qkv + ((size_t)i * T + t) * 3 * F;
            q[i] = ok ? ldc<E, TE>(row, c) : chunk_zero<E>();
            k[i] = ok ? ldc<E, TE>(row, nvec + c) : chunk_zero<E>();
            v[i] = ok ? ldc<E, TE>(row, 2 * nvec + c) : chunk_zero<E>();
        }
#pragma unroll
        for (int i = 0; i < S; ++i) {
            float sc[S], mx = -INFINITY;
#pragma unroll
            for (int j = 0; j < S; ++j) {
                sc[j] = group_sum(cdot<E>(q[i], k[j]), lph) * scale;
                mx = fmaxf(mx, sc[j]);
            }
            float den = 0.f;
#pragma unroll
            for (int j = 0; j < S; ++j) {
                sc[j] = expf(sc[j] - mx);
                den += sc[j];
            }
            const float inv = 1.0f / den;
            Chunk<E> o = chunk_zero<E>();
#pragma unroll
            for (int j = 0; j < S; ++j) {
                const float p = sc[j] * inv;
#pragma unroll
                for (int e = 0; e < E; ++e) o.v[e] += p * v[j].v[e];
            }
            if (ok) stc<E, TE>(out + ((size_t)i * T + t) * F, c, o);
        }
    }
}

template <int S, int E, typename TE>
__global__ __launch_bounds__(256) void seqattn_bwd_kernel_e(int T, int F, int dh, const TE* __restrict__ qkv, const TE* __restrict__ dout,
                                                            TE* __restrict__ dqkv) {
    const int lane = threadIdx.x & 63;
    const int t = (blockIdx.x * blockDim.x + threadIdx.x) >> 6;
    if (t >= T) return;
    const int nvec = F / E, lph = dh / E;
    const float scale = 1.0f / sqrtf((float)dh);
    for (int c0 = 0; c0 < nvec; c0 += 64) {
        const int c = c0 + lane;
        const bool ok = c < nvec;
        Chunk<E> q[S], k[S], v[S], go[S], dq[S], dk[S], dv[S];
#pragma unroll
        for (int i = 0; i < S; ++i) {
            const TE* row = qkv + ((size_t)i * T + t) * 3 * F;
            q[i] = ok ? ldc<E, TE>(row, c) : chunk_zero<E>();
            k[i] = ok ? ldc<E, TE>(row, nvec + c) : chunk_zero<E>();
            v[i] = ok ? ldc<E, TE>(row, 2 * nvec + c) : chunk_zero<E>();
            go[i] = ok ? ldc<E, TE>(dout + ((size_t)i * T + t) * F, c) : chunk_zero<E>();
            dq[i] = chunk_zero<E>(); dk[i] = chunk_zero<E>(); dv[i] = chunk_zero<E>();
        }
#pragma unroll
        for (int i = 0; i < S; ++i) {
// ... 303 lines not shown
    if constexpr (sizeof(TE) == 2) {
        if ((dh & 7) == 0 && pow2(dh / 8) &&
            ((reinterpret_cast<uintptr_t>(qkv) | reinterpret_cast<uintptr_t>(dout) | reinterpret_cast<uintptr_t>(dqkv)) & 15) == 0) {
            switch (s) {
                case 1: GRAPPA_LAUNCH((seqattn_bwd_kernel_e<1, 8, TE>), grid, dim3(256), 0, st, T, F, dh, qkv, dout, dqkv); break;
                case 2: GRAPPA_LAUNCH((seqattn_bwd_kernel_e<2, 8, TE>), grid, dim3(256), 0, st, T, F, dh, qkv, dout, dqkv); break;
                case 3: GRAPPA_LAUNCH((seqattn_bwd_kernel_e<3, 8, TE>), grid, dim3(256), 0, st, T, F, dh, qkv, dout, dqkv); break;
                default: GRAPPA_LAUNCH((seqattn_bwd_kernel_e<4, 8, TE>), grid, dim3(256), 0, st, T, F, dh, qkv, dout, dqkv); break;
            }
            return grappa_launch_status();
        }
    }
    switch (s) {
        case 1: GRAPPA_LAUNCH((seqattn_bwd_kernel<1, TE>), grid, dim3(256), 0, st, T, F, dh, qkv, dout, dqkv, row_amax); break;
        case 2: GRAPPA_LAUNCH((seqattn_bwd_kernel<2, TE>), grid, dim3(256), 0, st, T, F, dh, qkv, dout, dqkv, row_amax); break;
        case 3: GRAPPA_LAUNCH((seqattn_bwd_kernel<3, TE>), grid, dim3(256), 0, st, T, F, dh, qkv, dout, dqkv, row_amax); break;
        default: GRAPPA_LAUNCH((seqattn_bwd_kernel<4, TE>), grid, dim3(256), 0, st, T, F, dh, qkv, dout, dqkv, row_amax); break;
    }
    return grappa_launch_status();
}
}

extern "C" int grappa_tuple_gather_fwd_f32(void* stream, int T, int s, int W, const float* a, int lda, const int* idx, const float* pe,
                                           float* x, int ldx) {
    return tuple_gather_fwd_impl<float, float>(stream, T, s, W, a, lda, idx, pe, x, ldx);
}
extern "C" int grappa_tuple_gather_fwd_bf16(void* stream, int T, int s, int W, const uint16_t* a, int lda, const int* idx, const float* pe,
                                            uint16_t* x, int ldx) {
    return tuple_gather_fwd_impl<grappa_bf16_t, grappa_bf16_t>(stream, T, s, W, a, lda, idx, pe, x, ldx);
}
extern "C" int grappa_tuple_gather_bwd_f32(void* stream, int N, int W, const int* inv_ptr, const int* inv_rows, const float* dx, int lddx,
                                           float* da, int ldda, int has_pe, int accumulate) {
    return tuple_gather_bwd_impl<float, float>(stream, N, W, inv_ptr, inv_rows, dx, lddx, da, ldda, has_pe, accumulate);
}
extern "C" int grappa_tuple_gather_bwd_bf16(void* stream, int N, int W, const int* inv_ptr, const int* inv_rows, const uint16_t* dx, int lddx,
                                            uint16_t* da, int ldda, int has_pe, int accumulate) {
    return tuple_gather_bwd_impl<grappa_bf16_t, grappa_bf16_t>(stream, N, W, inv_ptr, inv_rows, dx, lddx, da, ldda, has_pe, accumulate);
}
namespace {
int seqattn_batch(const grappa_seqattn_item* items, int count, bool bwd, SeqAttnBatch& b) {
    if (!items || count <= 0 || count > GRAPPA_ROW_BATCH_MAX) return GRAPPA_ERR_ARG;
    b.count = count;
    b.blk_begin[0] = 0;
    for (int i = 0; i < count; ++i) {
        const grappa_seqattn_item& t = items[i];
        if (t.s < 1 || t.s > 4 || t.T < 0 || t.nheads <= 0 || t.dh <= 0 || (t.dh & 3) || !pow2(t.dh / 4) || t.dh / 4 > 64 || t.nheads * t.dh > 1024) return GRAPPA_ERR_ARG;
        if (t.T > 0) {
            if (!t.qkv || !aligned_el<float>(t.qkv)) return GRAPPA_ERR_ARG;
            if (bwd ? (!t.dout || !t.dqkv || !aligned_el<float>(t.dout) || !aligned_el<float>(t.dqkv)) : (!t.out || !aligned_el<float>(t.out))) return GRAPPA_ERR_ARG;
        }
        b.it[i] = t;
        b.blk_begin[i + 1] = b.blk_begin[i] + (t.T + 3) / 4;
    }
    for (int i = count; i < GRAPPA_ROW_BATCH_MAX; ++i) b.blk_begin[i + 1] = b.blk_begin[count];
    return GRAPPA_OK;
}
}

extern "C" int grappa_seqattn_fwd_batched_f32(void* stream, const grappa_seqattn_item* items, int count) {
    SeqAttnBatch b;
    const int rc = seqattn_batch(items, count, false, b);
    if (rc != GRAPPA_OK || b.blk_begin[count] == 0) return rc;
    GRAPPA_LAUNCH(seqattn_fwd_batched_kernel, dim3(b.blk_begin[count]), dim3(256), 0, reinterpret_cast<hipStream_t>(stream), b);
    return grappa_launch_status();
}
extern "C" int grappa_seqattn_bwd_batched_f32(void* stream, const grappa_seqattn_item* items, int count) {
    SeqAttnBatch b;
    const int rc = seqattn_batch(items, count, true, b);
    if (rc != GRAPPA_OK || b.blk_begin[count] == 0) return rc;
    GRAPPA_LAUNCH(seqattn_bwd_batched_kernel, dim3(b.blk_begin[count]), dim3(256), 0, reinterpret_cast<hipStream_t>(stream), b);
    return grappa_launch_status();
}

extern "C" int grappa_seqattn_fwd_f32(void* stream, int s, int T, int nheads, int dh, const float* qkv, float* out) {
    return seqattn_fwd_impl<float>(stream, s, T, nheads, dh, qkv, out);
}
extern "C" int grappa_seqattn_fwd_amax_f32(void* stream, int s, int T, int nheads, int dh, const float* qkv, float* out, uint32_t* out_amax) {
    return seqattn_fwd_impl<float>(stream, s, T, nheads, dh, qkv, out, out_amax);
}
extern "C" int grappa_seqattn_bwd_amax_f32(void* stream, int s, int T, int nheads, int dh, const float* qkv, const float* dout, float* dqkv,
                                           uint32_t* dqkv_amax) {
    return seqattn_bwd_impl<float>(stream, s, T, nheads, dh, qkv, dout, dqkv, dqkv_amax);
}
extern "C" int grappa_seqattn_fwd_pairs_f32(void* stream, int s, int T, int nheads, int dh, const float* qkv, uint16_t* pairs, int ldp,
                                            uint32_t* out_amax) {
    const int F = nheads * dh;
    if (s < 1 || s > 4 || T < 0 || nheads <= 0 || dh <= 0 || (dh & 3) || !pow2(dh / 4) || dh / 4 > 64 || F > 512 || (F & 31) || ldp < 2 * F || (ldp & 7))
        return GRAPPA_ERR_ARG;
    if (T == 0) return GRAPPA_OK;
    if (!qkv || !pairs || !out_amax || !aligned_el<float>(qkv) || (reinterpret_cast<uintptr_t>(pairs) & 15)) return GRAPPA_ERR_ARG;
    hipStream_t st = reinterpret_cast<hipStream_t>(stream);
    const dim3 grid((T + 3) / 4);
    switch (s) {
        case 1: GRAPPA_LAUNCH((seqattn_fwd_pairs_kernel<1>), grid, dim3(256), 0, st, T, F, dh, qkv, pairs, ldp, out_amax); break;
        case 2: GRAPPA_LAUNCH((seqattn_fwd_pairs_kernel<2>), grid, dim3(256), 0, st, T, F, dh, qkv, pairs, ldp, out_amax); break;
        case 3: GRAPPA_LAUNCH((seqattn_fwd_pairs_kernel<3>), grid, dim3(256), 0, st, T, F, dh, qkv, pairs, ldp, out_amax); break;
        default: GRAPPA_LAUNCH((seqattn_fwd_pairs_kernel<4>), grid, dim3(256), 0, st, T, F, dh, qkv, pairs, ldp, out_amax); break;
    }
    return grappa_launch_status();
}
extern "C" int grappa_seqattn_fwd_bf16(void* stream, int s, int T, int nheads, int dh, const uint16_t* qkv, uint16_t* out) {
    return seqattn_fwd_impl<grappa_bf16_t>(stream, s, T, nheads, dh, qkv, out);
}
extern "C" int grappa_seqattn_bwd_f32(void* stream, int s, int T, int nheads, int dh, const float* qkv, const float* dout, float* dqkv) {
    return seqattn_bwd_impl<float>(stream, s, T, nheads, dh, qkv, dout, dqkv);
}
extern "C" int grappa_seqattn_bwd_bf16(void* stream, int s, int T, int nheads, int dh, const uint16_t* qkv, const uint16_t* dout, uint16_t* dqkv) {
    return seqattn_bwd_impl<grappa_bf16_t>(stream, s, T, nheads, dh, qkv, dout, dqkv);
}

static int fill_perms(int s, int P, const int* h_perm, Perms& fwd, Perms& inv) {
    if (s < 1 || s > 4 || P < 1 || P > 6 || !h_perm) return GRAPPA_ERR_ARG;
    for (int p = 0; p < P; ++p) {
        int seen = 0;
        for (int j = 0; j < s; ++j) {
            const int v = h_perm[p * s + j];
            if (v < 0 || v >= s) return GRAPPA_ERR_ARG;
            fwd.p[p][j] = v;
            inv.p[p][v] = j;
            seen |= 1 << v;
        }
        if (seen != (1 << s) - 1) return GRAPPA_ERR_ARG;
    }
    return GRAPPA_OK;
}

namespace {
template <typename TE>
int perm_concat_fwd_impl(void* stream, int s, int T, int F, int P, const int* h_perm, const TE* x, TE* z) {
    Perms fwd, inv;
    if (int rc = fill_perms(s, P, h_perm, fwd, inv)) return rc;
    if (T < 0 || F <= 0 || (F & 3)) return GRAPPA_ERR_ARG;
    if (T == 0) return GRAPPA_OK;
    if (!x || !z || !aligned_el<TE>(x) || !aligned_el<TE>(z)) return GRAPPA_ERR_ARG;
    GRAPPA_LAUNCH(perm_concat_fwd_kernel<TE>, dim3(wave_grid((long)P * T * s)), dim3(256), 0, reinterpret_cast<hipStream_t>(stream), s, T, F, P,
                       fwd, x, z);
    return grappa_launch_status();
}
template <typename TE>
int perm_concat_bwd_impl(void* stream, int s, int T, int F, int P, const int* h_perm, const TE* dz, TE* dx) {
    Perms fwd, inv;
    if (int rc = fill_perms(s, P, h_perm, fwd, inv)) return rc;
    if (T < 0 || F <= 0 || (F & 3)) return GRAPPA_ERR_ARG;
    if (T == 0) return GRAPPA_OK;
    if (!dz || !dx || !aligned_el<TE>(dz) || !aligned_el<TE>(dx)) return GRAPPA_ERR_ARG;
    GRAPPA_LAUNCH(perm_concat_bwd_kernel<TE>, dim3(wave_grid((long)T * s)), dim3(256), 0, reinterpret_cast<hipStream_t>(stream), s, T, F, P, inv,
                       dz, dx);
    return grappa_launch_status();
}
}

extern "C" int grappa_perm_concat_fwd_f32(void* stream, int s, int T, int F, int P, const int* h_perm, const float* x, float* z) {
    return perm_concat_fwd_impl<float>(stream, s, T, F, P, h_perm, x, z);
}
extern "C" int grappa_perm_concat_fwd_bf16(void* stream, int s, int T, int F, int P, const int* h_perm, const uint16_t* x, uint16_t* z) {
    return perm_concat_fwd_impl<grappa_bf16_t>(stream, s, T, F, P, h_perm, x, z);
}
extern "C" int grappa_perm_concat_bwd_f32(void* stream, int s, int T, int F, int P, const int* h_perm, const float* dz, float* dx) {
    return perm_concat_bwd_impl<float>(stream, s, T, F, P, h_perm, dz, dx);
}
extern "C" int grappa_perm_concat_bwd_bf16(void* stream, int s, int T, int F, int P, const int* h_perm, const uint16_t* dz, uint16_t* dx) {
    return perm_concat_bwd_impl<grappa_bf16_t>(stream, s, T, F, P, h_perm, dz, dx);
}

extern "C" int grappa_param_out_fwd_f32(void* stream, int kind, int T, int P, int n_per, int gated, float cutoff, const float* o, int ldo,
                                        const float* consts, float* k, float* eq) {
    if (T < 0 || P < 1 || kind < 0 || kind > 2) return GRAPPA_ERR_ARG;
    if (kind == GRAPPA_OUT_TORSION && (n_per < 1 || ldo < (gated ? 2 : 1) * n_per)) return GRAPPA_ERR_ARG;
    if (kind != GRAPPA_OUT_TORSION && ldo < 2) return GRAPPA_ERR_ARG;
    if (T == 0) return GRAPPA_OK;
    if (!o || !consts || !k || (kind != GRAPPA_OUT_TORSION && !eq)) return GRAPPA_ERR_ARG;
    GRAPPA_LAUNCH(param_out_fwd_kernel, dim3((T + 255) / 256), dim3(256), 0, reinterpret_cast<hipStream_t>(stream), kind, T, P, n_per, gated,
                       cutoff, o, ldo, consts, k, eq);
    return grappa_launch_status();
}

extern "C" size_t grappa_param_out_stats_workspace_bytes(int T) {
    const int blocks = (T + 255) / 256 > 256 ? 256 : (T + 255) / 256;
    return (size_t)(blocks < 1 ? 1 : blocks) * STATS_MAX * sizeof(float);
}
// ... 27 lines not shown
```

### grappa_amd/ops.py

```python
from __future__ import annotations

import os
from typing import List, Optional, Sequence

import torch
from torch.autograd import Function

from .backend import get_backend
from .constants import TUPLE_LEVELS

ELU = 1
_SEED = {"base": 0x5DEECE66D, "counter": 0}


FIRST_LAYER_ON_ATOM_ROWS = os.environ.get("GRAPPA_FIRST_LAYER_ROWS", "1") not in ("0", "")


def manual_seed(seed: int) -> None:
    _SEED["base"] = int(seed) & (2 ** 63 - 1)
    _SEED["counter"] = 0


def next_seed() -> int:
    _SEED["counter"] += 1
# ... 306 lines not shown
        h = _c(h)
        N, Fd = h.shape
        h1, mean1, rstd1, sh1 = _ln_fwd(be, h, ln_w, ln_b)
        mn = _new((N, Fd), h)
        be.neighbor_mean(plan, h1, mn, False)
        t = _new((N, Fd), h, F32)
        smn = be.gemm(mn, w_neigh, t, M=N, N=Fd, K=Fd)
        y1 = _new((N, Fd), h)
        h3 = _new((N, Fd), h)
        sh1 = be.gemm(h1, w_self, y1, M=N, N=Fd, K=Fd, bias=bias, pre=t, act=ELU, drop_p=drop_p, drop_seed=seed1, res=h1, out2=h3, a_scales=sh1)
        if w is None:
            h4 = mean2 = rstd2 = y2 = sh4 = None
            out = h3
        else:
            h4, mean2, rstd2, sh4 = _ln_fwd(be, h3, ln2_w, ln2_b)
            y2 = _new((N, Fd), h)
            out = _new((N, Fd), h)
            sh4 = be.gemm(h4, w, y2, M=N, N=Fd, K=Fd, bias=b, act=ELU, drop_p=drop_p, drop_seed=seed2, res=h4, out2=out, a_scales=sh4)
        ctx.plan, ctx.cfg, ctx.scales = plan, (drop_p, seed1, seed2), (smn, sh1, sh4)
        ctx.save_for_backward(h, mean1, rstd1, h1, mn, y1, h3, mean2, rstd2, h4, y2, ln_w, ln_b, w_self, w_neigh, bias, ln2_w, ln2_b, w, b)
        return out

    @staticmethod
    def backward(ctx, dout):
        be = get_backend()
        (h, mean1, rstd1, h1, mn, y1, h3, mean2, rstd2, h4, y2, ln_w, ln_b, w_self, w_neigh, bias, ln2_w, ln2_b, w, b) = ctx.saved_tensors
        drop_p, seed1, seed2 = ctx.cfg
        plan = ctx.plan
        N, Fd = h.shape
        dout = _c(dout)
        smn, sh1, sh4 = ctx.scales
        if w is None:
            dh3 = dout
        else:
            dz2 = _new(dout.shape, dout)
            sz = be.act_dropout_bwd(dout, y2, drop_p, seed2, dz2)
            sz = _linear_bwd_params(be, dz2, h4, w, b, sh4, sz)
            dh4 = _new(h4.shape, h4)
            be.gemm(dz2, w, dh4, M=N, N=Fd, K=Fd, b_kcontig=False, res=dout, a_scales=sz)
            dh3, _ = _ln_bwd(be, dh4, h3, mean2, rstd2, ln2_w, ln2_b)
        dz1 = _new(dh3.shape, dh3)
        sz = be.act_dropout_bwd(dh3, y1, drop_p, seed1, dz1)
        sz = _linear_bwd_params(be, dz1, h1, w_self, bias, sh1, sz)
        sz = _linear_bwd_params(be, dz1, mn, w_neigh, None, smn, sz)
        dmn = _new(mn.shape, mn)
        be.gemm(dz1, w_neigh, dmn, M=N, N=Fd, K=Fd, b_kcontig=False, a_scales=sz)
        dh1 = _new(h1.shape, h1)
        if h1.dtype == F32:
            be.neighbor_mean(plan, dmn, dh1, True)
            be.gemm(dz1, w_self, dh1, M=N, N=Fd, K=Fd, b_kcontig=False, res=dh3, accumulate=True, a_scales=sz)
        else:
            agg = _new(h1.shape, h1, F32)
            be.neighbor_mean(plan, dmn, agg, True)
            be.gemm(dz1, w_self, dh1, M=N, N=Fd, K=Fd, b_kcontig=False, pre=agg, res=dh3, a_scales=sz)
        dh, _ = _ln_bwd(be, dh1, h, mean1, rstd1, ln_w, ln_b)
        _wgrads_aside(be)
        return (dh,) + (None,) * 13


class SplitHeadsFn(Function):

    @staticmethod
    def forward(ctx, h, n):
        ctx.set_materialize_grads(False)
        return tuple(h.view_as(h) for _ in range(n))

    @staticmethod
    def backward(ctx, *gs):
        be = get_backend()
        if getattr(be, "gnn_tails", False):
            be.set_tail_launches(True)
        _wgrads_aside(be, all_streams=True)
        gs = [_c(g) for g in gs if g is not None]
        if not gs:
            return None, None
        acc = gs[0]
        for g in gs[1:]:
            out = acc if acc is not gs[0] else torch.empty_like(acc)
            be.add(acc.reshape(-1), g.reshape(-1), out.reshape(-1))
            acc = out
        return acc, None


def _attention(be, qkv, s, T, nheads, like, infer):
    M, Fd = qkv.shape[0], qkv.shape[1] // 3
    if not T:
        return _new((M, Fd), like), None
    if infer and hasattr(be, "pairs_ok") and be.pairs_ok(qkv, Fd, training=infer == 2) and 32 < Fd <= 512 and M > 32:
        return None, be.seqattn_fwd(qkv, s, T, nheads, None, pairs=True)
    att = _new((M, Fd), like)
    return att, be.seqattn_fwd(qkv, s, T, nheads, att)


class ProjGatherFn(Function):

    @staticmethod
    def forward(ctx, h, w, b, idx32, inv_ptr, inv_rows, s, pe, out_dtype=None):
        be = get_backend()
        h = _c(h)
        N, R = h.shape
        Wp = w.shape[0]
        Fd = Wp + (1 if pe is not None else 0)
        T = idx32.shape[0]
        a = _zeros((N, Fd), h, out_dtype)
        ctx.sh = be.gemm(h, w, a[:, :Wp], M=N, N=Wp, K=R, bias=b, act=ELU)
        x = _new((s * T, Fd), a)
        if T:
            be.tuple_gather_fwd(a, idx32, s, pe, x)
        ctx.save_for_backward(h, w, b, a, inv_ptr, inv_rows)
        ctx.cfg = (s, T, Wp, pe is not None)
        return x

    @staticmethod
    def backward(ctx, dx):
        be = get_backend()
        h, w, b, a, inv_ptr, inv_rows = ctx.saved_tensors
        s, T, Wp, has_pe = ctx.cfg
        N, R = h.shape
        if T == 0:
            return (torch.zeros_like(h),) + (None,) * 8
        dx = _c(dx)
        da = _new(a.shape, a)
        be.tuple_gather_bwd(inv_ptr, inv_rows, dx, da, has_pe, False)
        dz = _padded_cols(N, Wp, a)
        sz = be.act_dropout_bwd(da[:, :Wp], a[:, :Wp], 0.0, 0, dz)
        sz = _linear_bwd_params(be, dz, h, w, b, ctx.sh, sz)
        dh = _new(h.shape, h)
        be.gemm(dz, w, dh, M=N, N=R, K=Wp, b_kcontig=False, a_scales=sz)
        return (dh,) + (None,) * 8


class TransformerLayerFn(Function):

    @staticmethod
    def forward(ctx, x, s, T, nheads, drop_p, seed1, seed2, n1_w, n1_b, w_in, b_in, w_o, b_o, nf_w, nf_b, w1, b1, w2, b2):
        be = get_backend()
        ctx.up_drop = getattr(x, "_grappa_drop", None)
        x = _c(x)
        M, Fd = x.shape
        infer = _infer(ctx)
        fused = getattr(be, "writer_layer_ok", None)
        if fused is not None and T and fused(x, s, nheads, n1_w, n1_b, w_in, b_in, w_o, b_o, nf_w, nf_b, w1, b1, w2, b2):
            out = _new((M, Fd), x)
            sv = None
            if infer != 1:
                tiled = bool(getattr(be, "fused_writer_layer_bwd", False))
                rows2 = be.lib.grappa_writer_head_tiles(s, T) * 64 if tiled else M
                sv = dict(mean1=_new((M,), x, F32), rstd1=_new((M,), x, F32), meanf=_new((M,), x, F32), rstdf=_new((M,), x, F32),
                          x1=_new((M, Fd), x), qkv=_new((M, 3 * Fd), x), att=_new((M, Fd), x), x2=_new((rows2, Fd), x), x3=_new((M, Fd), x),
                          u=_new((M, Fd), x), x2_tiled=tiled)
            be.writer_layer_fwd(x, s, T, nheads, drop_p, seed1, seed2, n1_w, n1_b, w_in, b_in, w_o, b_o, nf_w, nf_b, w1, b1, w2, b2, out, save=sv)
            ctx.cfg, ctx.scales = (s, T, nheads, drop_p, seed1, seed2), (None, None)
            ctx.fused_saved = sv if (sv is not None and sv.get("x2_tiled")) else None
            if sv is not None:
                ctx.ff_saved = (sv["x2"], sv["meanf"], sv["rstdf"], sv["x3"], sv["u"], None, None, None)
                ctx.save_for_backward(x, sv["mean1"], sv["rstd1"], sv["x1"], sv["qkv"], sv["att"], n1_w, n1_b, w_in, b_in, w_o, b_o, nf_w, nf_b, w1, b1, w2, b2)
            else:
                ctx.ff_saved = None
            if drop_p > 0:
                out._grappa_drop = (drop_p, seed2)
            return out
        lean = _pairs(be, x, infer) and n1_w is not None and M > 32 and Fd > 32
        x1, mean1, rstd1, sx1 = _ln_fwd(be, x, n1_w, n1_b, infer, need_y=not lean)
        qkv = _new((M, 3 * Fd), x)
        sx1 = be.gemm(x1, w_in, qkv, M=M, N=3 * Fd, K=Fd, bias=b_in, a_scales=sx1)
        att, satt = _attention(be, qkv, s, T, nheads, x, infer)
        x2 = _new((M, Fd), x)
        if x1 is None:
            satt = be.gemm(att, w_o, x2, M=M, N=Fd, K=Fd, bias=b_o, drop_p=drop_p, drop_seed=seed1, res=x, res_ln=(mean1, rstd1, n1_w, n1_b), a_scales=satt)
        else:
            satt = be.gemm(att, w_o, x2, M=M, N=Fd, K=Fd, bias=b_o, drop_p=drop_p, drop_seed=seed1, res=x1, a_scales=satt)
        out, ff_saved = _ff_fwd(be, x2, nf_w, nf_b, w1, b1, w2, b2, False, drop_p, seed2, True, infer)
        ctx.cfg, ctx.scales = (s, T, nheads, drop_p, seed1, seed2), (sx1, satt)
        ctx.ff_saved = ff_saved
        ctx.save_for_backward(x, mean1, rstd1, x1, qkv, att, n1_w, n1_b, w_in, b_in, w_o, b_o, nf_w, nf_b, w1, b1, w2, b2)
        if drop_p > 0:
            out._grappa_drop = (drop_p, seed2)
        return out

    @staticmethod
    def backward(ctx, dout):
        be = get_backend()
        x, mean1, rstd1, x1, qkv, att, n1_w, n1_b, w_in, b_in, w_o, b_o, nf_w, nf_b, w1, b1, w2, b2 = ctx.saved_tensors
        s, T, nheads, drop_p, seed1, seed2 = ctx.cfg
        M, Fd = x.shape
        if M == 0:
            return (torch.zeros_like(x),) + (None,) * 18
        sv = getattr(ctx, "fused_saved", None)
        if sv is not None:
            ctx.fused_saved = ctx.ff_saved = None
            dx, dz2, dz1, dzo, dqkv = be.writer_layer_bwd(_c(dout), x, s, T, nheads, drop_p, seed1, seed2, sv, n1_w, n1_b, w_in, w_o, nf_w, nf_b, w1, w2)
            _linear_bwd_params(be, dz2, sv["u"], w2, b2, None, None)
            _linear_bwd_params(be, dz1, sv["x3"], w1, b1, None, None)
            _linear_bwd_params(be, dzo, att, w_o, b_o, None, None)
            _linear_bwd_params(be, dqkv, x1, w_in, b_in, None, None)
            return (dx,) + (None,) * 18
        dx2, sz = _ff_bwd(be, ctx.ff_saved, dout, nf_w, nf_b, w1, b1, w2, b2, False, drop_p, seed2, True, then_drop=(drop_p, seed1))
        ctx.ff_saved = None
        dzo, sz = _drop_bwd(be, dx2, drop_p, seed1, w_o)
        sx1, satt = ctx.scales
        sz = _linear_bwd_params(be, dzo, att, w_o, b_o, satt, sz)
        datt = _new((M, Fd), x)
        be.gemm(dzo, w_o, datt, M=M, N=Fd, K=Fd, b_kcontig=False, a_scales=sz)
        dqkv = _new(qkv.shape, qkv)
        sz = be.seqattn_bwd(qkv, datt, s, T, nheads, dqkv)
        sz = _linear_bwd_params(be, dqkv, x1, w_in, b_in, sx1, sz)
        dx1 = _new(x.shape, x)
        be.gemm(dqkv, w_in, dx1, M=M, N=Fd, K=3 * Fd, b_kcontig=False, res=dx2, a_scales=sz)
        dx, _ = _ln_bwd(be, dx1, x, mean1, rstd1, n1_w, n1_b, drop=ctx.up_drop)
        return (dx,) + (None,) * 18


class ProjFirstLayerFn(Function):

    @staticmethod
    def forward(ctx, h, w, b, tabs, s, T, pe, out_dtype, nheads, drop_p, seed1, seed2, n1_w, n1_b, w_in, b_in, w_o, b_o, nf_w, nf_b, w1, b1, w2, b2):
        be = get_backend()
        idx_id, invid_ptr, invid_rows, idx_tab, invtab_ptr, invtab_rows = tabs
        h = _c(h)
        N, R = h.shape
        Wp = w.shape[0]
        Fd = Wp + (1 if pe is not None else 0)
        a = _zeros((N, Fd), h, out_dtype)
        sh = be.gemm(h, w, a[:, :Wp], M=N, N=Wp, K=R, bias=b, act=ELU)
        tab = _new((s * N, Fd), a)
        be.tuple_gather_fwd(a, idx_id, s, pe, tab)
        infer = _infer(ctx)
        x1_tab, mean1, rstd1, sx1 = _ln_fwd(be, tab, n1_w, n1_b, infer if infer == 1 else 0)
        qkv_tab = _new((s * N, 3 * Fd), tab)
        sx1 = be.gemm(x1_tab, w_in, qkv_tab, M=s * N, N=3 * Fd, K=Fd, bias=b_in, a_scales=sx1)
        M = s * T
        if hasattr(be, "credit"):
            be.credit("gemm_saved", 2.0 * (M - s * N) * 3 * Fd * Fd)
        fused = getattr(be, "writer_layer_ok", None)
        if fused is not None and fused(tab, s, nheads, n1_w, n1_b, w_in, b_in, w_o, b_o, nf_w, nf_b, w1, b1, w2, b2) and getattr(be, "fused_first_layer", True):
            out = _new((M, Fd), tab)
            sv = None
            if infer != 1:
                tiled = bool(getattr(be, "fused_writer_layer_bwd", False))
                rows2 = be.lib.grappa_writer_head_tiles(s, T) * 64 if tiled else M
                sv = dict(meanf=_new((M,), tab, F32), rstdf=_new((M,), tab, F32), att=_new((M, Fd), tab), x2=_new((rows2, Fd), tab), x3=_new((M, Fd), tab),
                          u=_new((M, Fd), tab), x2_tiled=tiled)
            be.writer_layer_fwd(None, s, T, nheads, drop_p, seed1, seed2, n1_w, n1_b, w_in, b_in, w_o, b_o, nf_w, nf_b, w1, b1, w2, b2, out, save=sv,
                                gather=(idx_tab, x1_tab, qkv_tab))
            ctx.cfg, ctx.scales = (s, T, N, Wp, pe is not None, nheads, drop_p, seed1, seed2), (sh, sx1, None)
            ctx.fused_saved = sv if (sv is not None and sv["x2_tiled"]) else None
            ctx.fused_gather = True
            if sv is not None:
                ctx.ff_saved = (sv["x2"], sv["meanf"], sv["rstdf"], sv["x3"], sv["u"], None, None, None)
                ctx.save_for_backward(h, a, tab, mean1, rstd1, x1_tab, qkv_tab, sv["att"], invid_ptr, invid_rows, invtab_ptr, invtab_rows,
                                      w, b, n1_w, n1_b, w_in, b_in, w_o, b_o, nf_w, nf_b, w1, b1, w2, b2, idx_tab)
            if drop_p > 0:
                out._grappa_drop = (drop_p, seed2)
            return out
        ctx.fused_gather = False
        x1, qkv = _new((M, Fd), tab), _new((M, 3 * Fd), tab)
        be.tuple_gather_fwd(x1_tab, idx_tab, s, None, x1)
        be.tuple_gather_fwd(qkv_tab, idx_tab, s, None, qkv)
        del qkv_tab
        att, satt = _attention(be, qkv, s, T, nheads, tab, infer)
        x2 = _new((M, Fd), tab)
        satt = be.gemm(att, w_o, x2, M=M, N=Fd, K=Fd, bias=b_o, drop_p=drop_p, drop_seed=seed1, res=x1, a_scales=satt)
        del x1
        out, ff_saved = _ff_fwd(be, x2, nf_w, nf_b, w1, b1, w2, b2, False, drop_p, seed2, True, infer)
        ctx.cfg, ctx.scales = (s, T, N, Wp, pe is not None, nheads, drop_p, seed1, seed2), (sh, sx1, satt)
        ctx.ff_saved = ff_saved
        ctx.save_for_backward(h, a, tab, mean1, rstd1, x1_tab, qkv, att, invid_ptr, invid_rows, invtab_ptr, invtab_rows,
                              w, b, n1_w, n1_b, w_in, b_in, w_o, b_o, nf_w, nf_b, w1, b1, w2, b2)
        if drop_p > 0:
            out._grappa_drop = (drop_p, seed2)
        return out

    @staticmethod
    def backward(ctx, dout):
        be = get_backend()
        idx_tab = None
        if getattr(ctx, "fused_gather", False):
            (h, a, tab, mean1, rstd1, x1_tab, qkv, att, invid_ptr, invid_rows, invtab_ptr, invtab_rows,
             w, b, n1_w, n1_b, w_in, b_in, w_o, b_o, nf_w, nf_b, w1, b1, w2, b2, idx_tab) = ctx.saved_tensors
        else:
            (h, a, tab, mean1, rstd1, x1_tab, qkv, att, invid_ptr, invid_rows, invtab_ptr, invtab_rows,
             w, b, n1_w, n1_b, w_in, b_in, w_o, b_o, nf_w, nf_b, w1, b1, w2, b2) = ctx.saved_tensors
        s, T, N, Wp, has_pe, nheads, drop_p, seed1, seed2 = ctx.cfg
        sh, sx1, satt = ctx.scales
        M, Fd = s * T, qkv.shape[1] // 3
        R = h.shape[1]
        sv = getattr(ctx, "fused_saved", None)
        if idx_tab is not None and sv is not None:
            ctx.fused_saved = ctx.ff_saved = None
            dx2, dz2, dz1, dzo, dqkv = be.writer_layer_bwd(_c(dout), None, s, T, nheads, drop_p, seed1, seed2, sv, n1_w, n1_b, w_in, w_o, nf_w, nf_b, w1, w2,
                                                           gather=(idx_tab, qkv))
            _linear_bwd_params(be, dz2, sv["u"], w2, b2, None, None)
            _linear_bwd_params(be, dz1, sv["x3"], w1, b1, None, None)
            _linear_bwd_params(be, dzo, att, w_o, b_o, None, None)
        else:
            if idx_tab is not None:
                qkv_tok = _new((M, 3 * Fd), tab)
                be.tuple_gather_fwd(qkv, idx_tab, s, None, qkv_tok)
                qkv = qkv_tok
            dx2, sz = _ff_bwd(be, ctx.ff_saved, dout, nf_w, nf_b, w1, b1, w2, b2, False, drop_p, seed2, True, then_drop=(drop_p, seed1))
            ctx.ff_saved = None
            dzo, sz = _drop_bwd(be, dx2, drop_p, seed1, w_o)
            sz = _linear_bwd_params(be, dzo, att, w_o, b_o, satt, sz)
            datt = _new((M, Fd), qkv)
            be.gemm(dzo, w_o, datt, M=M, N=Fd, K=Fd, b_kcontig=False, a_scales=sz)
            dqkv = _new(qkv.shape, qkv)
            be.seqattn_bwd(qkv, datt, s, T, nheads, dqkv)
        dqkv_tab, dres_tab = _new((s * N, 3 * Fd), qkv), _new((s * N, Fd), qkv)
        be.tuple_gather_bwd(invtab_ptr, invtab_rows, dqkv, dqkv_tab, False, False)
        be.tuple_gather_bwd(invtab_ptr, invtab_rows, dx2, dres_tab, False, False)
        del dqkv
        sz = _linear_bwd_params(be, dqkv_tab, x1_tab, w_in, b_in, sx1, None)
        if hasattr(be, "credit"):
            be.credit("gemm_saved", 2.0 * 2.0 * (M - s * N) * 3 * Fd * Fd)
        dx1_tab = _new(x1_tab.shape, x1_tab)
        be.gemm(dqkv_tab, w_in, dx1_tab, M=s * N, N=Fd, K=3 * Fd, b_kcontig=False, res=dres_tab, a_scales=sz)
        dtab, _ = _ln_bwd(be, dx1_tab, tab, mean1, rstd1, n1_w, n1_b)
        da = _new(a.shape, a)
        be.tuple_gather_bwd(invid_ptr, invid_rows, dtab, da, has_pe, False)
        dz = _padded_cols(N, Wp, a)
        sz = be.act_dropout_bwd(da[:, :Wp], a[:, :Wp], 0.0, 0, dz)
        sz = _linear_bwd_params(be, dz, h, w, b, sh, sz)
        dh = _new(h.shape, h)
        be.gemm(dz, w, dh, M=N, N=R, K=Wp, b_kcontig=False, a_scales=sz)
        return (dh,) + (None,) * 23


class SymmetriserFn(Function):

    @staticmethod
    def forward(ctx, x, s, T, perms, n_layers, *params):
        be = get_backend()
        x = _c(x)
        Fd = x.shape[1]
        P = len(perms)
        layers = [params[6 * i:6 * i + 6] for i in range(n_layers)]
        z = _new((P * T, s * Fd), x)
        if T:
            be.perm_concat_fwd(x, s, T, perms, z)
        saved = []
        cur = z
        for i, (nw, nb, w1, b1, w2, b2) in enumerate(layers):
            skip = (i != 0) and (i != n_layers - 1)
            cur, sv = _ff_fwd(be, cur, nw, nb, w1, b1, w2, b2, False, 0.0, 0, skip, _infer(ctx))
            saved.append(sv)
        ctx.cfg = (s, T, perms, n_layers, tuple(x.shape), x.dtype)
        ctx.saved_layers = saved
        ctx.layers = layers
        return cur

    @staticmethod
    def backward(ctx, dout):
        be = get_backend()
        s, T, perms, n_layers, xshape, xdtype = ctx.cfg
        nret = 5 + 6 * n_layers
        if T == 0:
            return (torch.zeros(xshape, dtype=xdtype, device=dout.device),) + (None,) * (nret - 1)
        g, sg = _c(dout), None
        for i in reversed(range(n_layers)):
            nw, nb, w1, b1, w2, b2 = ctx.layers[i]
            skip = (i != 0) and (i != n_layers - 1)
            g, sg = _ff_bwd(be, ctx.saved_layers[i], g, nw, nb, w1, b1, w2, b2, False, 0.0, 0, skip, sg)
        ctx.saved_layers = None
        dx = torch.empty(xshape, dtype=xdtype, device=dout.device)
        be.perm_concat_bwd(g, s, T, perms, dx)
        return (dx,) + (None,) * (nret - 1)


class ParamOutFn(Function):

    @staticmethod
    def forward(ctx, o, kind, T, P, n_per, gated, cutoff, consts):
        be = get_backend()
        o = _c(o)
        if kind == 2:
            k = _new((T, n_per), o)
            eq = None
        else:
            k, eq = _new((T,), o), _new((T,), o)
        if T:
            be.param_out_fwd(kind, o, T, P, n_per, gated, cutoff, consts, k, eq)
        ctx.save_for_backward(o, consts)
        ctx.cfg = (kind, T, P, n_per, gated, cutoff)
        if kind == 2:
            return k
        return k, eq

    @staticmethod
    def backward(ctx, dk, deq=None):
        be = get_backend()
        o, consts = ctx.saved_tensors
        kind, T, P, n_per, gated, cutoff = ctx.cfg
        d_o = _new(o.shape, o)
        dk = _c(dk) if dk is not None else None
        deq = _c(deq) if deq is not None else None
# ... 370 lines not shown
```

### grappa_amd/trainer.py

```python
from __future__ import annotations

import os
import time
from typing import Dict, List, Optional, Sequence, Union

import numpy as np
import torch
import torch.distributed as tdist

from .device_dataset import DeviceDataset, ShapeBuckets
from .dist import BucketedGradReducer, shard_indices
from .energy import Energy
from .evaluation import Evaluator, FastEvaluator
from .loss import MolwiseLoss
from .optim import FlatParams, FusedAdam
from .schedule import TrainSchedule


def epoch_batches(names: List[str], batch_size: int, shuffle: bool = True, weights: Dict[str, float] = {}, balance_factor: float = 0.,
                  generator: Optional[torch.Generator] = None, min_last: int = 1, sizes: Optional[Sequence[int]] = None,
                  size_window: int = 0) -> List[np.ndarray]:
    n = len(names)
    assert 0 <= balance_factor <= 1, f"balance_factor must be between 0 and 1, but got {balance_factor}"
    if shuffle and (len(weights) or balance_factor > 0):
# ... 21 lines not shown
            pool = np.concatenate(full)
            pool = pool[np.argsort(-sz[pool], kind="stable")]
            lanes = [[] for _ in full]
            for r in range(0, len(pool), len(full)):
                chunk = pool[r:r + len(full)]
                idx = range(len(chunk)) if (r // len(full)) % 2 == 0 else range(len(full) - 1, len(full) - 1 - len(chunk), -1)
                for lane, m in zip(idx, chunk):
                    lanes[lane].append(m)
            it = iter(lanes)
            for i, b in enumerate(group):
                if len(b) == batch_size:
                    batches[w0 + i] = np.asarray(next(it), dtype=order.dtype)
    if len(batches) > 1 and len(batches[-1]) < min_last:
        tail = batches.pop()
        batches[-1] = np.concatenate([batches[-1], tail])
    if batches and len(batches[-1]) < min_last:
        raise ValueError(f"{n} molecules cannot be dealt to {min_last} ranks")
    return batches


class Trainer:
    def __init__(self, model, train_set: DeviceDataset, val_set: Optional[DeviceDataset] = None, batch_size: int = 32,
                 conf_strategy: Union[str, int] = 32, val_batch_size: int = 32, val_conf_strategy: Union[str, int] = "max",
                 lr: float = 1.5e-5, weight_decay: float = 0., gradient_clip_val: Optional[float] = 10.0,
                 proper_regularisation: float = 1e-3, improper_regularisation: float = 0., param_weights_by_dataset: Dict[str, float] = {},
                 weights: Dict[str, float] = {}, balance_factor: float = 0., seed: int = 0, size_window: int = 0, recorded: bool = False,
                 shape_buckets: int = 4, max_recorded_steps: int = 16, pipelined: bool = True, **schedule_kwargs):
        self.model, self.train_set, self.val_set = model, train_set, val_set
        self.recorded, self.shape_buckets, self.max_recorded_steps = bool(recorded), int(shape_buckets), int(max_recorded_steps)
        self._buckets: Optional[ShapeBuckets] = None
        self._steps: Dict[tuple, object] = {}
        self._prep_stream, self._load_done = None, None
        self._unrecordable: Dict[tuple, str] = {}
        self._val_buckets: Optional[ShapeBuckets] = None
        self._test_buckets: Dict[tuple, ShapeBuckets] = {}
        self._eval_steps: Dict[tuple, object] = {}
        self.pipelined, self._prep_pool = bool(pipelined), None
        self.recorded_stats = {"replayed": 0, "eager": 0, "graphs_recorded": 0, "padding_rows": 0, "real_rows": 0}
        self._graphs_off = False
        self.batch_size, self.conf_strategy = batch_size, conf_strategy
        self.val_batch_size, self.val_conf_strategy = val_batch_size, val_conf_strategy
        self.weights, self.balance_factor = dict(weights), balance_factor
        self.size_window = int(size_window)
        self.schedule = TrainSchedule(lr=lr, **schedule_kwargs)
        self.loss_fn = MolwiseLoss(proper_regularisation=proper_regularisation, improper_regularisation=improper_regularisation,
                                   param_weights_by_dataset=param_weights_by_dataset, **self.schedule.initial_loss_weights())
        self.energy = Energy()
        self.flat = FlatParams(model)
        self.opt = FusedAdam(self.flat, lr=lr, weight_decay=weight_decay, max_grad_norm=gradient_clip_val)
        self.reducer = BucketedGradReducer(model, self.flat)
        self.evaluator = FastEvaluator()
        self.gen = torch.Generator().manual_seed(seed)
        self.world = tdist.get_world_size() if tdist.is_available() and tdist.is_initialized() else 1
        self.rank = tdist.get_rank() if self.world > 1 else 0
        self.history: List[Dict] = []
        self.next_epoch = 0

    def _my_share(self, ids: np.ndarray) -> np.ndarray:
        if self.world == 1:
            return ids
        sizes = self.train_set.count["n1"][ids]
        return ids[shard_indices(sizes.tolist(), self.world, self.rank)]

    def train_step(self, ids: np.ndarray) -> torch.Tensor:
        self.opt.lr = self.schedule.next_lr()
        mine = self._my_share(np.asarray(ids))
        g, names = self.train_set.collate(mine, self.conf_strategy)
        self.loss_fn.global_batch_size = len(ids) if self.world > 1 else None
        self.opt.zero_grad()
        loss = self.loss_fn(self.energy(self.model(g)), list(names))
        loss.backward()
        self.reducer.finish()
        self.opt.step()
        return loss.detach()

    def _step_stamp(self) -> tuple:
        lf, o = self.loss_fn, self.opt
        from . import ops
        from .backend import get_backend
        be = get_backend()
        pw = getattr(self.model, "parameter_writer", None)
        backend_cfg = tuple(getattr(be, k, None) for k in ("gemm_precision_name", "gemm_precision_bwd_name", "inference_pairs", "training_pairs", "backward_pairs",
                                                            "_tails", "plan_override", "splitk_reduce", "weight_pairs_min_rows", "pairs_min_rows",
                                                            "fused_writer_layer", "fused_writer_layer_bwd", "group_launches", "wgrads_aside"))
        return (float(lf.gradient_weight), float(lf.energy_weight), float(lf.param_weight), float(lf.tuplewise_weight), float(lf.proper_regularisation),
                float(lf.improper_regularisation), tuple(sorted(lf.weights.items())), tuple(sorted(lf.param_weights_by_dataset.items())),
                tuple(o.betas), float(o.eps), float(o.weight_decay), o.max_grad_norm, bool(self.model.training), backend_cfg,
                str(ops.act_dtype()), getattr(pw, "head_streams", None), getattr(pw, "merged_heads", None))

    def calibrate_buckets(self, batches: Sequence[np.ndarray]) -> ShapeBuckets:
        self._buckets = ShapeBuckets(self.train_set, batches, n_buckets=self.shape_buckets)
        self.train_set.enable_padding(self._buckets.max_pad)
        return self._buckets

    def _prepare_padded(self, ids: np.ndarray, caps, tot):
        dev = self.train_set.device
        if self._prep_stream is None:
            self._prep_stream = torch.cuda.Stream(device=dev)
            self._prep_stream.wait_stream(torch.cuda.current_stream(dev))
        side = self._prep_stream
        if self._load_done is not None:
            side.wait_event(self._load_done)
        with torch.cuda.stream(side):
            g, names = self.train_set.collate(ids, self.conf_strategy, pad_to=caps)
            plan = g.plan()
            plan.param_weight_rows = self.loss_fn.param_weights_of(list(names), plan.B).pin_memory().to(plan.device, non_blocking=True)
            for lvl in ("n2", "n3", "n4", "n4_improper"):
                if plan.T[lvl]:
                    plan.position_tables(lvl)
            ready = torch.cuda.Event()
            ready.record(side)
        return g, names, ready

    def _prepare(self, ids: np.ndarray):
        ids = self._my_share(np.asarray(ids))
        tot = self.train_set.totals(ids)
        caps = self._buckets.choose(tot) if self._buckets is not None else None
        if caps is None or any(caps[k] - tot[k] > self.train_set.pad_caps[k] for k in tot):
            return None
        if self.train_set.device.type == "cuda" and self.train_set.device.index is not None:
            torch.cuda.set_device(self.train_set.device)
        return self._prepare_padded(ids, caps, tot) + (tot, caps)

    def train_step_recorded(self, ids: np.ndarray, prepared="unset", after_load=None) -> torch.Tensor:
        from .capture import CapturedTrainStep, train_signature
        ids = np.asarray(ids)
        if isinstance(prepared, str):
            prepared = self._prepare(ids)
        if prepared is None:
            self.recorded_stats["eager"] += 1
            if self._prep_stream is not None:
                torch.cuda.current_stream(self.train_set.device).wait_stream(self._prep_stream)
                self._prep_stream.wait_stream(torch.cuda.current_stream(self.train_set.device))
            loss = self.train_step(ids)
            if after_load is not None:
                after_load()
            return loss
        lr = self.schedule.next_lr()
        g, names, ready, tot, caps = prepared
        main = torch.cuda.current_stream(self.train_set.device)
        main.wait_event(ready)
        self.loss_fn.global_batch_size = len(ids) if self.world > 1 else None
        reducer = self.reducer if self.world > 1 else None
        key = (train_signature(g), self._step_stamp(), self.loss_fn.global_batch_size)
        step = self._steps.pop(key, None) if key not in self._unrecordable else None
        if step is None and key not in self._unrecordable:
            if len(self._steps) >= self.max_recorded_steps:
                old = self._steps.pop(next(iter(self._steps)))
                self._release(old)
            try:
                step = CapturedTrainStep(self.model, self.energy, self.loss_fn, self.opt, g, preserve_state=True, static_inputs=True, reducer=reducer)
                self.recorded_stats["graphs_recorded"] += 1
            except Exception as e:
                import warnings
                self._unrecordable[key] = repr(e)
                warnings.warn(f"Trainer(recorded=True): recording a train step failed ({e!r}); batches of this shape run eagerly")
                step = None
        elif step is not None:
            try:
                step.load(g)
            except Exception as e:
                import warnings
                warnings.warn(f"Trainer(recorded=True): a batch did not fit its recorded step ({e!r}); it runs eagerly")
                self._steps[key] = step
                step = None
        if step is None:
            self.recorded_stats["eager"] += 1
# ... 237 lines not shown
```

### include/grappa_hip.h

```cpp
#ifndef GRAPPA_HIP_H
#define GRAPPA_HIP_H

#include <stddef.h>
#include <stdint.h>

#ifdef __cplusplus
extern "C" {
#endif

#define GRAPPA_OK 0
#define GRAPPA_ERR_ARG (-1)
#define GRAPPA_ERR_LAUNCH (-2)
#define GRAPPA_ERR_WORKSPACE (-3)

#define GRAPPA_ABI_VERSION 11
int grappa_abi_version(void);
const char* grappa_build_arch(void);
long long grappa_launch_count(int reset);

#define GRAPPA_ACT_NONE 0
#define GRAPPA_ACT_ELU 1

#define GRAPPA_GEMM_F32_MFMA 0
#define GRAPPA_GEMM_F32_BF16X9 1
// ... 74 lines not shown
int grappa_act_dropout_bwd_f32(void* stream, int M, int N, const float* dy, int lddy, const float* y, int ldy,
                               float drop_p, uint64_t drop_seed, float* dz, int lddz, const uint64_t* drop_salt);
int grappa_act_dropout_bwd_amax_f32(void* stream, int M, int N, const float* dy, int lddy, const float* y, int ldy,
                                    float drop_p, uint64_t drop_seed, float* dz, int lddz, uint32_t* dz_amax, const uint64_t* drop_salt);
#define GRAPPA_ROW_BATCH_MAX 4
typedef struct grappa_ln_fwd_item {
    int M, W; const float* x; int ldx; const float* gamma; const float* beta; float* y; int ldy; float* mean; float* rstd; uint32_t* y_amax;
} grappa_ln_fwd_item;
int grappa_layernorm_fwd_batched_f32(void* stream, const grappa_ln_fwd_item* items, int count);
typedef struct grappa_ln_bwd_item {
    int M, W; const float* dy; int lddy; const float* x; int ldx; const float* mean; const float* rstd; const float* gamma; float* dx; int lddx;
    float* part; uint32_t* dx_amax;
} grappa_ln_bwd_item;
int grappa_layernorm_bwd_batched_f32(void* stream, const grappa_ln_bwd_item* items, int count);
typedef struct grappa_act_dropout_item {
    int M, N; const float* dy; int lddy; const float* y; int ldy; float drop_p; uint64_t drop_seed; float* dz; int lddz; uint32_t* dz_amax;
    const uint64_t* drop_salt;
} grappa_act_dropout_item;
int grappa_act_dropout_bwd_batched_f32(void* stream, const grappa_act_dropout_item* items, int count);
typedef struct grappa_seqattn_item {
    int s, T, nheads, dh; const float* qkv; float* out; const float* dout; float* dqkv; uint32_t* amax;
} grappa_seqattn_item;
int grappa_seqattn_fwd_batched_f32(void* stream, const grappa_seqattn_item* items, int count);
int grappa_seqattn_bwd_batched_f32(void* stream, const grappa_seqattn_item* items, int count);
int grappa_act_dropout_bwd_pairs_f32(void* stream, int M, int N, const float* dy, int lddy, const float* y, int ldy, float drop_p,
                                     uint64_t drop_seed, float* dz, int lddz, uint32_t* dz_amax, uint16_t* pairs, int ldp, const uint64_t* drop_salt);

int grappa_add_f32(void* stream, size_t n, const float* x, const float* z, float* y);

int grappa_layernorm_fwd_f32(void* stream, int M, int W, const float* x, int ldx, const float* gamma, const float* beta,
                             float* y, int ldy, float* mean, float* rstd);
int grappa_layernorm_fwd_amax_f32(void* stream, int M, int W, const float* x, int ldx, const float* gamma, const float* beta,
                                  float* y, int ldy, float* mean, float* rstd, uint32_t* y_amax);
int grappa_layernorm_fwd_pairs_f32(void* stream, int M, int W, const float* x, int ldx, const float* gamma, const float* beta,
                                   float* y, int ldy, float* mean, float* rstd, uint32_t* y_amax, uint16_t* pairs, int ldp);
size_t grappa_layernorm_bwd_workspace_bytes(int M, int W);
int grappa_layernorm_bwd_partial_rows(int M);
typedef struct {
    const float* part;
    int nrows, n;
    float* out;
    float* out2;
    int n_first;
    int accumulate;
} grappa_colsum_item;
int grappa_colsum_partials_batched(void* stream, const grappa_colsum_item* items, int count);
int grappa_layernorm_bwd_f32(void* stream, int M, int W, const float* dy, int lddy, const float* x, int ldx,
                             const float* mean, const float* rstd, const float* gamma,
                             float* dx, int lddx, float* dgamma, float* dbeta, int accumulate,
                             void* ws, size_t ws_bytes);
int grappa_layernorm_bwd_amax_f32(void* stream, int M, int W, const float* dy, int lddy, const float* x, int ldx,
                                  const float* mean, const float* rstd, const float* gamma,
                                  float* dx, int lddx, float* dgamma, float* dbeta, int accumulate,
                                  void* ws, size_t ws_bytes, uint32_t* dx_amax);
int grappa_layernorm_bwd_drop_f32(void* stream, int M, int W, const float* dy, int lddy, const float* x, int ldx,
                                  const float* mean, const float* rstd, const float* gamma,
                                  float* dx, int lddx, float* dgamma, float* dbeta, int accumulate,
                                  void* ws, size_t ws_bytes, uint32_t* dx_amax,
                                  float drop_p, uint64_t drop_seed, float* dz, int lddz, uint32_t* dz_amax, const uint64_t* drop_salt);

int grappa_gat_fwd_f32(void* stream, int N, int E, int H, int D, const int* indptr, const int* indices,
                       const float* ft, float* out, float* alpha);
int grappa_gat_bwd_f32(void* stream, int N, int E, int H, int D, const int* indptr, const int* indices, const int* rev,
                       const float* ft, const float* out, const float* alpha, const float* dout,
                       float* dft, float* delta );
int grappa_neighbor_mean_f32(void* stream, int N, int F, const int* indptr, const int* indices,
                             const float* x, float* out, int scale_by_neighbor);
int grappa_neighbor_mean_bf16(void* stream, int N, int F, const int* indptr, const int* indices,
                              const uint16_t* x, void* out, int out_f32, int scale_by_neighbor);

int grappa_charge_encoding_f32(void* stream, int N, const float* q, int dim, float lo, float hi, float* out, int ldo, int col0);

int grappa_tuple_gather_fwd_f32(void* stream, int T, int s, int W, const float* a, int lda, const int* idx,
                                const float* pe, float* x, int ldx);
int grappa_tuple_gather_bwd_f32(void* stream, int N, int W, const int* inv_ptr, const int* inv_rows,
                                const float* dx, int lddx, float* da, int ldda, int has_pe, int accumulate);

int grappa_seqattn_fwd_f32(void* stream, int s, int T, int nheads, int dh, const float* qkv, float* out);
int grappa_seqattn_bwd_f32(void* stream, int s, int T, int nheads, int dh, const float* qkv, const float* dout, float* dqkv);
int grappa_seqattn_fwd_amax_f32(void* stream, int s, int T, int nheads, int dh, const float* qkv, float* out, uint32_t* out_amax);
int grappa_seqattn_fwd_pairs_f32(void* stream, int s, int T, int nheads, int dh, const float* qkv, uint16_t* pairs, int ldp, uint32_t* out_amax);
int grappa_seqattn_bwd_amax_f32(void* stream, int s, int T, int nheads, int dh, const float* qkv, const float* dout, float* dqkv,
                                uint32_t* dqkv_amax);

int grappa_perm_concat_fwd_f32(void* stream, int s, int T, int F, int P, const int* h_perm, const float* x, float* z);
int grappa_perm_concat_bwd_f32(void* stream, int s, int T, int F, int P, const int* h_perm, const float* dz, float* dx);

#define GRAPPA_OUT_BOND 0
#define GRAPPA_OUT_ANGLE 1
#define GRAPPA_OUT_TORSION 2
int grappa_param_out_fwd_f32(void* stream, int kind, int T, int P, int n_per, int gated, float cutoff,
                             const float* o, int ldo, const float* consts, float* k, float* eq);
int grappa_param_out_bwd_f32(void* stream, int kind, int T, int P, int n_per, int gated, float cutoff,
                             const float* o, int ldo, const float* consts, const float* dk, const float* deq,
                             float* d_o);
size_t grappa_param_out_stats_workspace_bytes(int T);
int grappa_param_out_bwd_stats_f32(void* stream, int kind, int T, int P, int n_per, int gated, float cutoff, const float* o, int ldo,
                                   const float* consts, const float* dk, const float* deq, float* d_consts, void* ws, size_t ws_bytes);

typedef struct grappa_mm_desc {
    int N, C, B;
    const float* xyz;
    int T[4];
    const int* idx[4];
    const float* k[4];
    const float* eq[4];
    const int* mol_ptr[4];
    int n_per[4];
    int offset_torsion;
    const int* inc_ptr;
    const int* inc_code;
    const int* atom_molptr;
} grappa_mm_desc;

int grappa_mm_energy_fwd_f32(void* stream, const grappa_mm_desc* d, float* energy, float* term_energy,
                             float* const tuple_e[4], float* const tuple_x[4]);
int grappa_mm_gradient_fwd_f32(void* stream, const grappa_mm_desc* d, float* grad);
int grappa_mm_bwd_f32(void* stream, const grappa_mm_desc* d, const float* gE, const float* gG,
                      float* const gk[4], float* const geq[4]);

#define GRAPPA_NB_IBLOCK 64
typedef struct grappa_nb_desc {
    int N, C, B;
    const float* xyz;
    const int*   atom_molptr;
    const float *charge, *sigma, *epsilon;
    const int*   exc_ptr;
    const int*   exc_atom;
    const float *exc_qq, *exc_sigma, *exc_eps;
} grappa_nb_desc;
int grappa_nonbonded_iblock(void);
size_t grappa_nonbonded_workspace_bytes(int N, int C, int B);
int grappa_nonbonded_fwd_f32(void* stream, const grappa_nb_desc* d, float* energy , float* term_energy ,
                             float* grad , void* ws, size_t ws_bytes);
long long grappa_nonbonded_plan(int N, int C, int B, const int* atom_molptr_host, int* table, long long table_ints);
int grappa_nonbonded_fwd_planned_f32(void* stream, const grappa_nb_desc* d, const int* table_dev, int n_items, int n_blocks, float* energy,
                                     float* term_energy, float* grad, void* ws, size_t ws_bytes);

typedef struct grappa_relax_opts {
    float tolerance;
    int   max_steps;
    float dt_start, dt_max, max_disp;
    int   n_min;
    float f_inc, f_dec, alpha_start, f_alpha;
} grappa_relax_opts;
int grappa_relax_max_atoms(void);
int grappa_relax_fire_f32(void* stream, const grappa_mm_desc* mm, const grappa_nb_desc* nb, const grappa_relax_opts* o, float* xyz_out,
                          float* energy, float* term_energy, float* grad, float* gmax, int* steps, int* status);

size_t grappa_relax_steps_workspace_bytes(int N, int C, int B, int n_blocks);
int grappa_relax_steps_init_f32(void* stream, const grappa_mm_desc* mm, const grappa_nb_desc* nb, const grappa_relax_opts* o,
                                const int* table_dev, int n_items, int n_blocks, void* ws, size_t ws_bytes, int* n_running_dev);
int grappa_relax_steps_run_f32(void* stream, const grappa_mm_desc* mm, const grappa_nb_desc* nb, const grappa_relax_opts* o,
                               const int* table_dev, int n_items, int n_blocks, void* ws, size_t ws_bytes, int n_steps, int* n_running_dev);
int grappa_relax_steps_finish_f32(void* stream, const grappa_mm_desc* mm, const grappa_nb_desc* nb, const grappa_relax_opts* o,
                                  const int* table_dev, int n_items, int n_blocks, void* ws, size_t ws_bytes, float* xyz_out, float* energy,
                                  float* term_energy, float* grad, float* gmax, int* steps, int* status);

typedef struct grappa_md_opts {
    float dt;
    float temperature;
    float friction;
    float init_temperature;
    int   n_steps, save_every;
    unsigned first_step;
} grappa_md_opts;
// ... 130 lines not shown
```

Before: 7569.

## Index qkv table directly in first-layer attention and fuse dual gather backward

The first-layer attention kernels (forward, pairs forward, backward) now read q/k/v rows through a per-tuple row index into the per-atom table. This avoids materialising the gathered (s*T, 3F) qkv tensor in forward and regathering it in backward. The two tuple-gather backward launches (dqkv and residual) are merged into one kernel that also emits row amax for the following weight-gradient GEMM. The cost is more indirect, scattered reads inside the attention kernels and more code paths to keep consistent.

```diff
diff --git a/grappa_amd/_lib.py b/grappa_amd/_lib.py
--- a/grappa_amd/_lib.py
+++ b/grappa_amd/_lib.py
@@ -180,6 +180,10 @@
     "grappa_seqattn_bwd_f32": (_i, [_vp, _i, _i, _i, _i, _vp, _vp, _vp]),
     "grappa_seqattn_fwd_amax_f32": (_i, [_vp, _i, _i, _i, _i, _vp, _vp, _vp]),
     "grappa_seqattn_bwd_amax_f32": (_i, [_vp, _i, _i, _i, _i, _vp, _vp, _vp, _vp]),
+    "grappa_seqattn_fwd_idx_f32": (_i, [_vp, _i, _i, _i, _i, _vp, _vp, _vp, _vp]),
+    "grappa_seqattn_fwd_pairs_idx_f32": (_i, [_vp, _i, _i, _i, _i, _vp, _vp, _vp, _i, _vp]),
+    "grappa_seqattn_bwd_idx_f32": (_i, [_vp, _i, _i, _i, _i, _vp, _vp, _vp, _vp, _vp]),
+    "grappa_tuple_gather_bwd2_f32": (_i, [_vp, _i, _vp, _vp, _i, _i, _i, _vp, _i, _vp, _i, _vp, _i, _vp, _i, _vp, _i, _vp]),
     "grappa_perm_concat_fwd_f32": (_i, [_vp, _i, _i, _i, _i, c_int_p, _vp, _vp]),
     "grappa_perm_concat_bwd_f32": (_i, [_vp, _i, _i, _i, _i, c_int_p, _vp, _vp]),
     "grappa_param_out_fwd_f32": (_i, [_vp, _i, _i, _i, _i, _i, _f, _vp, _i, _vp, _vp, _vp]),
diff --git a/grappa_amd/backend.py b/grappa_amd/backend.py
--- a/grappa_amd/backend.py
+++ b/grappa_amd/backend.py
@@ -170,6 +170,7 @@
         self.fused_writer_layer = os.environ.get("GRAPPA_FUSED_WRITER_LAYER", "1") not in ("0", "")
         self.fused_writer_layer_bwd = os.environ.get("GRAPPA_FUSED_WRITER_LAYER_BWD", "1") not in ("0", "")
         self.fused_first_layer = os.environ.get("GRAPPA_FUSED_FIRST_LAYER", "1") not in ("0", "")
+        self.first_layer_indexed = os.environ.get("GRAPPA_FIRST_LAYER_INDEXED", "1") not in ("0", "")
         self._wplanes = {}
         self._wpairs = {}
         self._wptable = None
@@ -1294,7 +1295,7 @@
         _chk(fn(self._stream(), T, s, W, a.data_ptr(), _f32_2d(a, "a", dev, dt), idx.data_ptr(), _ptr(pe),
                 x.data_ptr(), _f32_2d(x, "x", dev, dt)), "grappa_tuple_gather_fwd")
 
-    def tuple_gather_bwd(self, inv_ptr, inv_rows, dx, da, has_pe: bool, accumulate=False) -> None:
+    def tuple_gather_bwd(self, inv_ptr, inv_rows, dx, da, has_pe: bool, accumulate=False, amax=False, second=None):
         dev = da.device
         N, W = da.shape[0], dx.shape[1]
         if inv_ptr.dtype != torch.int32 or inv_ptr.numel() != N + 1 or inv_ptr.device != dev or inv_rows.dtype != torch.int32:
@@ -1302,21 +1303,48 @@
         if da.shape[1] < W or inv_rows.numel() != dx.shape[0]:
             raise ValueError("tuple_gather_bwd: shapes")
         dt = _same_dtype(dx, da)
+        if self.first_layer_indexed and da.dtype == torch.float32:
+            row = self._new_row_amax(da, True, None if amax is None else bool(amax))
+            W2 = ld2x = ld2a = 0
+            dx2 = da2 = None
+            if second is not None:
+                dx2, da2 = second
+                W2 = dx2.shape[1]
+                if da2.shape[0] != N or da2.shape[1] < W2 or dx2.shape[0] != dx.shape[0] or _same_dtype(dx2, da2) != dt:
+                    raise ValueError("tuple_gather_bwd: shapes of the second table")
+                ld2x, ld2a = _f32_2d(dx2, "dx2", dev, dt), _f32_2d(da2, "da2", dev, dt)
+            _chk(self.lib.grappa_tuple_gather_bwd2_f32(self._stream(), N, inv_ptr.data_ptr(), inv_rows.data_ptr(), int(has_pe), int(accumulate),
+                                                       W, dx.data_ptr(), _f32_2d(dx, "dx", dev, dt), da.data_ptr(), _f32_2d(da, "da", dev, dt), _ptr(row),
+                                                       W2, _ptr(dx2), ld2x, _ptr(da2), ld2a, None), "grappa_tuple_gather_bwd2_f32")
+            return Amax(row=row) if row is not None else None
         fn = getattr(self.lib, f"grappa_tuple_gather_bwd_{_sfx(da)}")
-        _chk(fn(self._stream(), N, W, inv_ptr.data_ptr(), inv_rows.data_ptr(), dx.data_ptr(),
-                _f32_2d(dx, "dx", dev, dt), da.data_ptr(), _f32_2d(da, "da", dev, dt), int(has_pe), int(accumulate)),
-             "grappa_tuple_gather_bwd")
-
-    def seqattn_fwd(self, qkv, s, T, nheads, out, amax=None, pairs=False):
+        for x_, a_ in ((dx, da),) + ((second,) if second is not None else ()):
+            _chk(fn(self._stream(), N, x_.shape[1], inv_ptr.data_ptr(), inv_rows.data_ptr(), x_.data_ptr(),
+                    _f32_2d(x_, "dx", dev, dt), a_.data_ptr(), _f32_2d(a_, "da", dev, dt), int(has_pe), int(accumulate)),
+                 "grappa_tuple_gather_bwd")
+        return None
+
+    def _row_index(self, row_idx, s, T, qkv, table_rows, who):
+        if row_idx.dtype != torch.int32 or row_idx.device != qkv.device or not row_idx.is_contiguous() or tuple(row_idx.shape) != (T, s):
+            raise ValueError(f"{who}: row_idx must be contiguous int32 (T,s)")
+        if qkv.dtype != torch.float32 or (table_rows is not None and qkv.shape[0] != table_rows):
+            raise ValueError(f"{who}: the indexed q | k | v table must be float32 of table_rows rows")
+
+    def seqattn_fwd(self, qkv, s, T, nheads, out, amax=None, pairs=False, row_idx=None, table_rows=None):
+        if row_idx is not None:
+            self._row_index(row_idx, s, T, qkv, table_rows, "seqattn_fwd")
         if pairs:
             dev = qkv.device
             F = qkv.shape[1] // 3
-            if qkv.dtype != torch.float32 or qkv.shape != (s * T, 3 * F) or F % nheads or F % 32 or F > 512:
+            if qkv.dtype != torch.float32 or qkv.shape[1] != 3 * F or (row_idx is None and qkv.shape[0] != s * T) or F % nheads or F % 32 or F > 512:
                 raise ValueError("seqattn_fwd: the pair format needs float32 q, k, v of F % 32 == 0, F <= 512 columns each")
             _flat(qkv, "qkv", dev)
             row = torch.empty(s * T, dtype=torch.int32, device=dev)
             pr = torch.empty((s * T, 2 * F), dtype=torch.float16, device=dev)
-            if T:
+            if T and row_idx is not None:
+                _chk(self.lib.grappa_seqattn_fwd_pairs_idx_f32(self._stream(), s, T, nheads, F // nheads, qkv.data_ptr(), row_idx.data_ptr(), pr.data_ptr(),
+                                                               pr.stride(0), row.data_ptr()), "grappa_seqattn_fwd_pairs_idx_f32")
+            elif T:
                 _chk(self.lib.grappa_seqattn_fwd_pairs_f32(self._stream(), s, T, nheads, F // nheads, qkv.data_ptr(), pr.data_ptr(), pr.stride(0),
                                                            row.data_ptr()), "grappa_seqattn_fwd_pairs_f32")
             return Amax(row=row, pairs=pr)
@@ -1324,9 +1352,13 @@
         dt = _same_dtype(qkv, out)
         _flat(qkv, "qkv", dev, dt), _flat(out, "out", dev, dt)
         F = out.shape[1]
-        if qkv.shape != (s * T, 3 * F) or out.shape[0] != s * T or F % nheads:
+        if qkv.shape[1] != 3 * F or (row_idx is None and qkv.shape[0] != s * T) or out.shape[0] != s * T or F % nheads:
             raise ValueError("seqattn_fwd: shapes")
         row = self._new_row_amax(out, False, amax)
+        if row_idx is not None:
+            _chk(self.lib.grappa_seqattn_fwd_idx_f32(self._stream(), s, T, nheads, F // nheads, qkv.data_ptr(), row_idx.data_ptr(), out.data_ptr(),
+                                                     _ptr(row)), "grappa_seqattn_fwd_idx_f32")
+            return Amax(row=row) if row is not None else None
         args = (self._stream(), s, T, nheads, F // nheads, qkv.data_ptr(), out.data_ptr())
         if row is not None:
             _chk(self.lib.grappa_seqattn_fwd_amax_f32(*args, row.data_ptr()), "grappa_seqattn_fwd_amax_f32")
@@ -1474,14 +1506,20 @@
         a.part, a.nrows, a.n, a.out, a.out2, a.n_first, a.accumulate = part.data_ptr(), nrows, 2 * W, dg.data_ptr(), db.data_ptr(), W, 1
         _chk(self.lib.grappa_colsum_partials_batched(self._stream(), arr, 1), "grappa_colsum_partials_batched")
 
-    def seqattn_bwd(self, qkv, dout, s, T, nheads, dqkv, amax=None):
+    def seqattn_bwd(self, qkv, dout, s, T, nheads, dqkv, amax=None, row_idx=None):
         dev = dqkv.device
         dt = _same_dtype(qkv, dout, dqkv)
         _flat(qkv, "qkv", dev, dt), _flat(dout, "dout", dev, dt), _flat(dqkv, "dqkv", dev, dt)
         F = dout.shape[1]
-        if qkv.shape != (s * T, 3 * F) or dqkv.shape != qkv.shape or dout.shape[0] != s * T:
+        if row_idx is not None:
+            self._row_index(row_idx, s, T, qkv, None, "seqattn_bwd")
+        if qkv.shape[1] != 3 * F or (row_idx is None and qkv.shape[0] != s * T) or tuple(dqkv.shape) != (s * T, 3 * F) or dout.shape[0] != s * T:
             raise ValueError("seqattn_bwd: shapes")
         row = self._new_row_amax(dqkv, True, amax)
+        if row_idx is not None:
+            _chk(self.lib.grappa_seqattn_bwd_idx_f32(self._stream(), s, T, nheads, F // nheads, qkv.data_ptr(), row_idx.data_ptr(), dout.data_ptr(),
+                                                     dqkv.data_ptr(), _ptr(row)), "grappa_seqattn_bwd_idx_f32")
+            return Amax(row=row) if row is not None else None
         args = (self._stream(), s, T, nheads, F // nheads, qkv.data_ptr(), dout.data_ptr(), dqkv.data_ptr())
         if row is not None:
             _chk(self.lib.grappa_seqattn_bwd_amax_f32(*args, row.data_ptr()), "grappa_seqattn_bwd_amax_f32")
diff --git a/grappa_amd/capture.py b/grappa_amd/capture.py
--- a/grappa_amd/capture.py
+++ b/grappa_amd/capture.py
@@ -292,7 +292,7 @@
         if ps is None:
             ps = self._params = list(self.model.parameters())
         return (be.gemm_precision_name, getattr(be, "gemm_precision_bwd", None), be.inference_pairs, be.training_pairs, be._tails, be.plan_override,
-                be.splitk_reduce, be.weight_pairs_min_rows, be.pairs_min_rows, tuple(p.data_ptr() for p in ps))
+                be.splitk_reduce, be.weight_pairs_min_rows, be.pairs_min_rows, getattr(be, "first_layer_indexed", None), tuple(p.data_ptr() for p in ps))
 
     def valid(self) -> bool:
         if self._config_stamp() != self.config_stamp:
diff --git a/grappa_amd/csrc/tuples.hip b/grappa_amd/csrc/tuples.hip
--- a/grappa_amd/csrc/tuples.hip
+++ b/grappa_amd/csrc/tuples.hip
@@ -60,12 +60,128 @@
     return v;
 }
 
-template <int S, typename TE>
+template <int NC>
+__device__ __forceinline__ unsigned gather_sum_cols(int lane, int r0, int r1, const int* __restrict__ inv_rows, const float* __restrict__ dx, int lddx,
+                                                    float* __restrict__ dst, int c0, int nvec, int has_pe, int accumulate) {
+    float4 acc[NC];
+    int cc[NC];
+    bool ok[NC], last[NC];
+#pragma unroll
+    for (int k = 0; k < NC; ++k) {
+        const int c = c0 + k * 64 + lane;
+        ok[k] = c < nvec;
+        cc[k] = min(c, nvec - 1);
+        last[k] = has_pe && cc[k] == nvec - 1;
+        acc[k] = accumulate ? ld4(dst, cc[k]) : make_float4(0.f, 0.f, 0.f, 0.f);
+    }
+    int j = r0;
+    for (; j + 4 <= r1; j += 4) {
+        int r[4];
+#pragma unroll
+        for (int u = 0; u < 4; ++u) r[u] = inv_rows[j + u];
+        float4 v[4][NC];
+#pragma unroll
+        for (int u = 0; u < 4; ++u) {
+            const float* src = dx + (size_t)r[u] * lddx;
+#pragma unroll
+            for (int k = 0; k < NC; ++k) v[u][k] = ld4(src, cc[k]);
+        }
+        __builtin_amdgcn_sched_barrier(0);
+#pragma unroll
+        for (int u = 0; u < 4; ++u) {
+#pragma unroll
+            for (int k = 0; k < NC; ++k) {
+                if (last[k]) v[u][k].w = 0.f;
+                acc[k].x += v[u][k].x; acc[k].y += v[u][k].y; acc[k].z += v[u][k].z; acc[k].w += v[u][k].w;
+            }
+        }
+    }
+    const int cnt = r1 - j;
+    if (cnt > 0) {
+        int r[3];
+#pragma unroll
+        for (int u = 0; u < 3; ++u) r[u] = inv_rows[u < cnt ? j + u : j];
+        float4 v[3][NC];
+#pragma unroll
+        for (int u = 0; u < 3; ++u) {
+            if (u < cnt) {
+                const float* src = dx + (size_t)r[u] * lddx;
+#pragma unroll
+                for (int k = 0; k < NC; ++k) v[u][k] = ld4(src, cc[k]);
+            }
+        }
+        __builtin_amdgcn_sched_barrier(0);
+#pragma unroll
+        for (int u = 0; u < 3; ++u) {
+            if (u < cnt) {
+#pragma unroll
+                for (int k = 0; k < NC; ++k) {
+                    if (last[k]) v[u][k].w = 0.f;
+                    acc[k].x += v[u][k].x; acc[k].y += v[u][k].y; acc[k].z += v[u][k].z; acc[k].w += v[u][k].w;
+                }
+            }
+        }
+    }
+    unsigned am = 0u;
+#pragma unroll
+    for (int k = 0; k < NC; ++k) {
+        if (ok[k]) {
+            st4(dst, c0 + k * 64 + lane, acc[k]);
+            if (last[k]) acc[k].w = 0.f;
+            am = max(am, mag4(acc[k]));
+        }
+    }
+    return am;
+}
+
+template <int NC>
+__device__ __forceinline__ void gather_sum_row(int lane, int n, int r0, int r1, const int* __restrict__ inv_rows, int W, const float* __restrict__ dx,
+                                               int lddx, float* __restrict__ da, int ldda, unsigned* __restrict__ row_amax, int has_pe, int accumulate) {
+    const int nvec = W >> 2;
+    float* dst = da + (size_t)n * ldda;
+    unsigned am = 0u;
+    for (int c0 = 0; c0 < nvec; c0 += NC * 64) am = max(am, gather_sum_cols<NC>(lane, r0, r1, inv_rows, dx, lddx, dst, c0, nvec, has_pe, accumulate));
+    if (row_amax) {
+        am = wave_umax(am);
+        if (lane == 0) row_amax[n] = am;
+    }
+}
+
+template <int NC, int NC2>
+__global__ __launch_bounds__(256) void tuple_gather_bwd2_kernel(int N, const int* __restrict__ inv_ptr, const int* __restrict__ inv_rows, int has_pe,
+                                                                int accumulate, int W, const float* __restrict__ dx, int lddx, float* __restrict__ da,
+                                                                int ldda, unsigned* __restrict__ da_amax, int W2, const float* __restrict__ dx2, int lddx2,
+                                                                float* __restrict__ da2, int ldda2, unsigned* __restrict__ da2_amax) {
+    const int lane = threadIdx.x & 63;
+    const int n = __builtin_amdgcn_readfirstlane((blockIdx.x * blockDim.x + threadIdx.x) >> 6);
+    if (n >= N) return;
+    const int r0 = inv_ptr[n], r1 = inv_ptr[n + 1];
+    gather_sum_row<NC>(lane, n, r0, r1, inv_rows, W, dx, lddx, da, ldda, da_amax, has_pe, accumulate);
+    if constexpr (NC2 > 0) gather_sum_row<NC2>(lane, n, r0, r1, inv_rows, W2, dx2, lddx2, da2, ldda2, da2_amax, has_pe, accumulate);
+}
+
+template <int S, bool IDX, typename TE>
+__device__ __forceinline__ void qkv_rows(const TE* __restrict__ qkv, const int* __restrict__ row_idx, int T, int t, int F, const TE* (&rows)[S]) {
+    if constexpr (IDX) {
+        int r[S];
+#pragma unroll
+        for (int i = 0; i < S; ++i) r[i] = __builtin_amdgcn_readfirstlane(row_idx[(size_t)t * S + i]);
+#pragma unroll
+        for (int i = 0; i < S; ++i) rows[i] = qkv + (size_t)r[i] * 3 * F;
+    } else {
+#pragma unroll
+        for (int i = 0; i < S; ++i) rows[i] = qkv + ((size_t)i * T + t) * 3 * F;
+    }
+}
+
+template <int S, typename TE, bool IDX = false>
 __device__ __forceinline__ void seqattn_fwd_body(int T, int F, int dh, const TE* __restrict__ qkv, TE* __restrict__ out,
-                                                 unsigned* __restrict__ row_amax, int vblock) {
+                                                 unsigned* __restrict__ row_amax, int vblock, const int* __restrict__ row_idx = nullptr) {
     const int lane = threadIdx.x & 63;
     const int t = (vblock * blockDim.x + threadIdx.x) >> 6;
     if (t >= T) return;
+    const TE* rows[S];
+    qkv_rows<S, IDX, TE>(qkv, row_idx, T, t, F, rows);
     const int nvec = F >> 2, lph = dh >> 2;
     const float scale = 1.0f / sqrtf((float)dh);
     unsigned am[S];
@@ -77,7 +193,7 @@
         float4 q[S], k[S], v[S];
 #pragma unroll
         for (int i = 0; i < S; ++i) {
-            const TE* row = qkv + ((size_t)i * T + t) * 3 * F;
+            const TE* row = rows[i];
             q[i] = ok ? ld4(row, c) : make_float4(0.f, 0.f, 0.f, 0.f);
             k[i] = ok ? ld4(row, nvec + c) : make_float4(0.f, 0.f, 0.f, 0.f);
             v[i] = ok ? ld4(row, 2 * nvec + c) : make_float4(0.f, 0.f, 0.f, 0.f);
@@ -122,6 +238,11 @@
 __global__ __launch_bounds__(256) void seqattn_fwd_kernel(int T, int F, int dh, const TE* __restrict__ qkv, TE* __restrict__ out,
                                                           unsigned* __restrict__ row_amax) {
     seqattn_fwd_body<S, TE>(T, F, dh, qkv, out, row_amax, blockIdx.x);
+}
+template <int S>
+__global__ __launch_bounds__(256) void seqattn_fwd_idx_kernel(int T, int F, int dh, const float* __restrict__ qkv_tab, const int* __restrict__ row_idx,
+                                                              float* __restrict__ out, unsigned* __restrict__ row_amax) {
+    seqattn_fwd_body<S, float, true>(T, F, dh, qkv_tab, out, row_amax, blockIdx.x, row_idx);
 }
 
 struct SeqAttnBatch {
@@ -142,12 +263,14 @@
     }
 }
 
-template <int S>
+template <int S, bool IDX = false>
 __global__ __launch_bounds__(256) void seqattn_fwd_pairs_kernel(int T, int F, int dh, const float* __restrict__ qkv, uint16_t* __restrict__ pairs, int ldp,
-                                                                unsigned* __restrict__ row_amax) {
+                                                                unsigned* __restrict__ row_amax, const int* __restrict__ row_idx) {
     const int lane = threadIdx.x & 63;
     const int t = (blockIdx.x * blockDim.x + threadIdx.x) >> 6;
     if (t >= T) return;
+    const float* rows[S];
+    qkv_rows<S, IDX, float>(qkv, row_idx, T, t, F, rows);
     const int nvec = F >> 2, lph = dh >> 2;
     const float scale = 1.0f / sqrtf((float)dh);
     unsigned am[S];
@@ -161,7 +284,7 @@
         float4 q[S], k[S], v[S];
 #pragma unroll
         for (int i = 0; i < S; ++i) {
-            const float* row = qkv + ((size_t)i * T + t) * 3 * F;
+            const float* row = rows[i];
             q[i] = ok ? ld4(row, c) : make_float4(0.f, 0.f, 0.f, 0.f);
             k[i] = ok ? ld4(row, nvec + c) : make_float4(0.f, 0.f, 0.f, 0.f);
             v[i] = ok ? ld4(row, 2 * nvec + c) : make_float4(0.f, 0.f, 0.f, 0.f);
@@ -205,12 +328,15 @@
     }
 }
 
-template <int S, typename TE>
+template <int S, typename TE, bool IDX = false>
 __device__ __forceinline__ void seqattn_bwd_body(int T, int F, int dh, const TE* __restrict__ qkv, const TE* __restrict__ dout,
-                                                 TE* __restrict__ dqkv, unsigned* __restrict__ row_amax, int vblock) {
+                                                 TE* __restrict__ dqkv, unsigned* __restrict__ row_amax, int vblock,
+                                                 const int* __restrict__ row_idx = nullptr) {
     const int lane = threadIdx.x & 63;
     const int t = (vblock * blockDim.x + threadIdx.x) >> 6;
     if (t >= T) return;
+    const TE* rows[S];
+    qkv_rows<S, IDX, TE>(qkv, row_idx, T, t, F, rows);
     const int nvec = F >> 2, lph = dh >> 2;
     const float scale = 1.0f / sqrtf((float)dh);
     const float4 zero = make_float4(0.f, 0.f, 0.f, 0.f);
@@ -223,7 +349,7 @@
         float4 q[S], k[S], v[S], go[S], dq[S], dk[S], dv[S];
 #pragma unroll
         for (int i = 0; i < S; ++i) {
-            const TE* row = qkv + ((size_t)i * T + t) * 3 * F;
+            const TE* row = rows[i];
             q[i] = ok ? ld4(row, c) : zero;
             k[i] = ok ? ld4(row, nvec + c) : zero;
             v[i] = ok ? ld4(row, 2 * nvec + c) : zero;
@@ -284,6 +410,11 @@
 __global__ __launch_bounds__(256) void seqattn_bwd_kernel(int T, int F, int dh, const TE* __restrict__ qkv, const TE* __restrict__ dout,
                                                           TE* __restrict__ dqkv, unsigned* __restrict__ row_amax) {
     seqattn_bwd_body<S, TE>(T, F, dh, qkv, dout, dqkv, row_amax, blockIdx.x);
+}
+template <int S>
+__global__ __launch_bounds__(256) void seqattn_bwd_idx_kernel(int T, int F, int dh, const float* __restrict__ qkv_tab, const int* __restrict__ row_idx,
+                                                              const float* __restrict__ dout, float* __restrict__ dqkv, unsigned* __restrict__ row_amax) {
+    seqattn_bwd_body<S, float, true>(T, F, dh, qkv_tab, dout, dqkv, row_amax, blockIdx.x, row_idx);
 }
 
 __global__ __launch_bounds__(256) void seqattn_bwd_batched_kernel(SeqAttnBatch b) {
@@ -753,20 +884,115 @@
                                            uint32_t* dqkv_amax) {
     return seqattn_bwd_impl<float>(stream, s, T, nheads, dh, qkv, dout, dqkv, dqkv_amax);
 }
-extern "C" int grappa_seqattn_fwd_pairs_f32(void* stream, int s, int T, int nheads, int dh, const float* qkv, uint16_t* pairs, int ldp,
-                                            uint32_t* out_amax) {
+namespace {
+int seqattn_fwd_pairs_impl(void* stream, int s, int T, int nheads, int dh, const float* qkv, const int* row_idx, bool indexed, uint16_t* pairs, int ldp,
+                           uint32_t* out_amax) {
     const int F = nheads * dh;
     if (s < 1 || s > 4 || T < 0 || nheads <= 0 || dh <= 0 || (dh & 3) || !pow2(dh / 4) || dh / 4 > 64 || F > 512 || (F & 31) || ldp < 2 * F || (ldp & 7))
         return GRAPPA_ERR_ARG;
+    if (indexed && !row_idx) return GRAPPA_ERR_ARG;
     if (T == 0) return GRAPPA_OK;
     if (!qkv || !pairs || !out_amax || !aligned_el<float>(qkv) || (reinterpret_cast<uintptr_t>(pairs) & 15)) return GRAPPA_ERR_ARG;
     hipStream_t st = reinterpret_cast<hipStream_t>(stream);
     const dim3 grid((T + 3) / 4);
+    if (indexed) {
+        switch (s) {
+            case 1: GRAPPA_LAUNCH((seqattn_fwd_pairs_kernel<1, true>), grid, dim3(256), 0, st, T, F, dh, qkv, pairs, ldp, out_amax, row_idx); break;
+            case 2: GRAPPA_LAUNCH((seqattn_fwd_pairs_kernel<2, true>), grid, dim3(256), 0, st, T, F, dh, qkv, pairs, ldp, out_amax, row_idx); break;
+            case 3: GRAPPA_LAUNCH((seqattn_fwd_pairs_kernel<3, true>), grid, dim3(256), 0, st, T, F, dh, qkv, pairs, ldp, out_amax, row_idx); break;
+            default: GRAPPA_LAUNCH((seqattn_fwd_pairs_kernel<4, true>), grid, dim3(256), 0, st, T, F, dh, qkv, pairs, ldp, out_amax, row_idx); break;
+        }
+        return grappa_launch_status();
+    }
     switch (s) {
-        case 1: GRAPPA_LAUNCH((seqattn_fwd_pairs_kernel<1>), grid, dim3(256), 0, st, T, F, dh, qkv, pairs, ldp, out_amax); break;
-        case 2: GRAPPA_LAUNCH((seqattn_fwd_pairs_kernel<2>), grid, dim3(256), 0, st, T, F, dh, qkv, pairs, ldp, out_amax); break;
-        case 3: GRAPPA_LAUNCH((seqattn_fwd_pairs_kernel<3>), grid, dim3(256), 0, st, T, F, dh, qkv, pairs, ldp, out_amax); break;
-        default: GRAPPA_LAUNCH((seqattn_fwd_pairs_kernel<4>), grid, dim3(256), 0, st, T, F, dh, qkv, pairs, ldp, out_amax); break;
+        case 1: GRAPPA_LAUNCH((seqattn_fwd_pairs_kernel<1>), grid, dim3(256), 0, st, T, F, dh, qkv, pairs, ldp, out_amax, (const int*)nullptr); break;
+        case 2: GRAPPA_LAUNCH((seqattn_fwd_pairs_kernel<2>), grid, dim3(256), 0, st, T, F, dh, qkv, pairs, ldp, out_amax, (const int*)nullptr); break;
+        case 3: GRAPPA_LAUNCH((seqattn_fwd_pairs_kernel<3>), grid, dim3(256), 0, st, T, F, dh, qkv, pairs, ldp, out_amax, (const int*)nullptr); break;
+        default: GRAPPA_LAUNCH((seqattn_fwd_pairs_kernel<4>), grid, dim3(256), 0, st, T, F, dh, qkv, pairs, ldp, out_amax, (const int*)nullptr); break;
+    }
+    return grappa_launch_status();
+}
+
+bool seqattn_shape_ok(int s, int T, int nheads, int dh) {
+    return !(s < 1 || s > 4 || T < 0 || nheads <= 0 || dh <= 0 || (dh & 3) || !pow2(dh / 4) || dh / 4 > 64 || nheads * dh > 1024);
+}
+
+inline int gather_chunks(int W) {
+    const int n = ((W >> 2) + 63) / 64;
+    return n <= 4 ? n : 6;
+}
+template <int NC>
+void launch_gather_bwd2(hipStream_t st, int N, const int* inv_ptr, const int* inv_rows, int has_pe, int accumulate, int W, const float* dx, int lddx,
+                        float* da, int ldda, uint32_t* da_amax, int W2, const float* dx2, int lddx2, float* da2, int ldda2, uint32_t* da2_amax) {
+    const dim3 grid((N + 3) / 4);
+#define GRAPPA_GB2(NC2)                                                                                                                           \
+    GRAPPA_LAUNCH((tuple_gather_bwd2_kernel<NC, NC2>), grid, dim3(256), 0, st, N, inv_ptr, inv_rows, has_pe, accumulate, W, dx, lddx, da, ldda, \
+                  da_amax, W2, dx2, lddx2, da2, ldda2, da2_amax)
+    switch (W2 > 0 ? gather_chunks(W2) : 0) {
+        case 0: GRAPPA_GB2(0); break;
+        case 1:
+        case 2: GRAPPA_GB2(2); break;
+        default: GRAPPA_GB2(6); break;
+    }
+#undef GRAPPA_GB2
+}
+}
+
+extern "C" int grappa_seqattn_fwd_pairs_f32(void* stream, int s, int T, int nheads, int dh, const float* qkv, uint16_t* pairs, int ldp,
+                                            uint32_t* out_amax) {
+    return seqattn_fwd_pairs_impl(stream, s, T, nheads, dh, qkv, nullptr, false, pairs, ldp, out_amax);
+}
+extern "C" int grappa_seqattn_fwd_pairs_idx_f32(void* stream, int s, int T, int nheads, int dh, const float* qkv_tab, const int* row_idx,
+                                                uint16_t* pairs, int ldp, uint32_t* out_amax) {
+    return seqattn_fwd_pairs_impl(stream, s, T, nheads, dh, qkv_tab, row_idx, true, pairs, ldp, out_amax);
+}
+extern "C" int grappa_seqattn_fwd_idx_f32(void* stream, int s, int T, int nheads, int dh, const float* qkv_tab, const int* row_idx, float* out,
+                                          uint32_t* out_amax) {
+    if (!seqattn_shape_ok(s, T, nheads, dh) || !row_idx) return GRAPPA_ERR_ARG;
+    if (T == 0) return GRAPPA_OK;
+    if (!qkv_tab || !out || !aligned_el<float>(qkv_tab) || !aligned_el<float>(out)) return GRAPPA_ERR_ARG;
+    hipStream_t st = reinterpret_cast<hipStream_t>(stream);
+    const dim3 grid((T + 3) / 4);
+    const int F = nheads * dh;
+    switch (s) {
+        case 1: GRAPPA_LAUNCH((seqattn_fwd_idx_kernel<1>), grid, dim3(256), 0, st, T, F, dh, qkv_tab, row_idx, out, out_amax); break;
+        case 2: GRAPPA_LAUNCH((seqattn_fwd_idx_kernel<2>), grid, dim3(256), 0, st, T, F, dh, qkv_tab, row_idx, out, out_amax); break;
+        case 3: GRAPPA_LAUNCH((seqattn_fwd_idx_kernel<3>), grid, dim3(256), 0, st, T, F, dh, qkv_tab, row_idx, out, out_amax); break;
+        default: GRAPPA_LAUNCH((seqattn_fwd_idx_kernel<4>), grid, dim3(256), 0, st, T, F, dh, qkv_tab, row_idx, out, out_amax); break;
+    }
+    return grappa_launch_status();
+}
+extern "C" int grappa_seqattn_bwd_idx_f32(void* stream, int s, int T, int nheads, int dh, const float* qkv_tab, const int* row_idx, const float* dout,
+                                          float* dqkv, uint32_t* dqkv_amax) {
+    if (!seqattn_shape_ok(s, T, nheads, dh) || !row_idx) return GRAPPA_ERR_ARG;
+    if (T == 0) return GRAPPA_OK;
+    if (!qkv_tab || !dout || !dqkv || !aligned_el<float>(qkv_tab) || !aligned_el<float>(dout) || !aligned_el<float>(dqkv)) return GRAPPA_ERR_ARG;
+    hipStream_t st = reinterpret_cast<hipStream_t>(stream);
+    const dim3 grid((T + 3) / 4);
+    const int F = nheads * dh;
+    switch (s) {
+        case 1: GRAPPA_LAUNCH((seqattn_bwd_idx_kernel<1>), grid, dim3(256), 0, st, T, F, dh, qkv_tab, row_idx, dout, dqkv, dqkv_amax); break;
+        case 2: GRAPPA_LAUNCH((seqattn_bwd_idx_kernel<2>), grid, dim3(256), 0, st, T, F, dh, qkv_tab, row_idx, dout, dqkv, dqkv_amax); break;
+        case 3: GRAPPA_LAUNCH((seqattn_bwd_idx_kernel<3>), grid, dim3(256), 0, st, T, F, dh, qkv_tab, row_idx, dout, dqkv, dqkv_amax); break;
+        default: GRAPPA_LAUNCH((seqattn_bwd_idx_kernel<4>), grid, dim3(256), 0, st, T, F, dh, qkv_tab, row_idx, dout, dqkv, dqkv_amax); break;
+    }
+    return grappa_launch_status();
+}
+extern "C" int grappa_tuple_gather_bwd2_f32(void* stream, int N, const int* inv_ptr, const int* inv_rows, int has_pe, int accumulate, int W,
+                                            const float* dx, int lddx, float* da, int ldda, uint32_t* da_amax, int W2, const float* dx2, int lddx2,
+                                            float* da2, int ldda2, uint32_t* da2_amax) {
+    if (N < 0 || W <= 0 || (W & 3) || (lddx & 3) || (ldda & 3) || lddx < W || ldda < W) return GRAPPA_ERR_ARG;
+    if (W2 < 0 || (W2 > 0 && ((W2 & 3) || (lddx2 & 3) || (ldda2 & 3) || lddx2 < W2 || ldda2 < W2))) return GRAPPA_ERR_ARG;
+    if (N == 0) return GRAPPA_OK;
+    if (!inv_ptr || !da || !aligned_el<float>(da) || (dx && !aligned_el<float>(dx))) return GRAPPA_ERR_ARG;
+    if (W2 > 0 && (!da2 || !aligned_el<float>(da2) || (dx2 && !aligned_el<float>(dx2)))) return GRAPPA_ERR_ARG;
+    hipStream_t st = reinterpret_cast<hipStream_t>(stream);
+    switch (gather_chunks(W)) {
+        case 1: launch_gather_bwd2<1>(st, N, inv_ptr, inv_rows, has_pe, accumulate, W, dx, lddx, da, ldda, da_amax, W2, dx2, lddx2, da2, ldda2, da2_amax); break;
+        case 2: launch_gather_bwd2<2>(st, N, inv_ptr, inv_rows, has_pe, accumulate, W, dx, lddx, da, ldda, da_amax, W2, dx2, lddx2, da2, ldda2, da2_amax); break;
+        case 3: launch_gather_bwd2<3>(st, N, inv_ptr, inv_rows, has_pe, accumulate, W, dx, lddx, da, ldda, da_amax, W2, dx2, lddx2, da2, ldda2, da2_amax); break;
+        case 4: launch_gather_bwd2<4>(st, N, inv_ptr, inv_rows, has_pe, accumulate, W, dx, lddx, da, ldda, da_amax, W2, dx2, lddx2, da2, ldda2, da2_amax); break;
+        default: launch_gather_bwd2<6>(st, N, inv_ptr, inv_rows, has_pe, accumulate, W, dx, lddx, da, ldda, da_amax, W2, dx2, lddx2, da2, ldda2, da2_amax); break;
     }
     return grappa_launch_status();
 }
diff --git a/grappa_amd/ops.py b/grappa_amd/ops.py
--- a/grappa_amd/ops.py
+++ b/grappa_amd/ops.py
@@ -412,14 +412,16 @@
         return acc, None
 
 
-def _attention(be, qkv, s, T, nheads, like, infer):
-    M, Fd = qkv.shape[0], qkv.shape[1] // 3
+def _attention(be, qkv, s, T, nheads, like, infer, row_idx=None):
+    M, Fd = qkv.shape[0] if row_idx is None else s * T, qkv.shape[1] // 3
     if not T:
         return _new((M, Fd), like), None
-    if infer and hasattr(be, "pairs_ok") and be.pairs_ok(qkv, Fd, training=infer == 2) and 32 < Fd <= 512 and M > 32:
-        return None, be.seqattn_fwd(qkv, s, T, nheads, None, pairs=True)
+    kw = {} if row_idx is None else dict(row_idx=row_idx, table_rows=qkv.shape[0])
+    tok = qkv if row_idx is None else qkv[:1].expand(M, -1)
+    if infer and hasattr(be, "pairs_ok") and be.pairs_ok(tok, Fd, training=infer == 2) and 32 < Fd <= 512 and M > 32:
+        return None, be.seqattn_fwd(qkv, s, T, nheads, None, pairs=True, **kw)
     att = _new((M, Fd), like)
-    return att, be.seqattn_fwd(qkv, s, T, nheads, att)
+    return att, be.seqattn_fwd(qkv, s, T, nheads, att, **kw)
 
 
 class ProjGatherFn(Function):
@@ -584,11 +586,17 @@
                 out._grappa_drop = (drop_p, seed2)
             return out
         ctx.fused_gather = False
-        x1, qkv = _new((M, Fd), tab), _new((M, 3 * Fd), tab)
+        ctx.indexed = indexed = bool(getattr(be, "first_layer_indexed", False)) and qkv_tab.dtype == F32 and T > 0
+        x1 = _new((M, Fd), tab)
         be.tuple_gather_fwd(x1_tab, idx_tab, s, None, x1)
-        be.tuple_gather_fwd(qkv_tab, idx_tab, s, None, qkv)
+        if indexed:
+            qkv = qkv_tab
+            att, satt = _attention(be, qkv_tab, s, T, nheads, tab, infer, row_idx=idx_tab)
+        else:
+            qkv = _new((M, 3 * Fd), tab)
+            be.tuple_gather_fwd(qkv_tab, idx_tab, s, None, qkv)
+            att, satt = _attention(be, qkv, s, T, nheads, tab, infer)
         del qkv_tab
-        att, satt = _attention(be, qkv, s, T, nheads, tab, infer)
         x2 = _new((M, Fd), tab)
         satt = be.gemm(att, w_o, x2, M=M, N=Fd, K=Fd, bias=b_o, drop_p=drop_p, drop_seed=seed1, res=x1, a_scales=satt)
         del x1
@@ -596,7 +604,7 @@
         ctx.cfg, ctx.scales = (s, T, N, Wp, pe is not None, nheads, drop_p, seed1, seed2), (sh, sx1, satt)
         ctx.ff_saved = ff_saved
         ctx.save_for_backward(h, a, tab, mean1, rstd1, x1_tab, qkv, att, invid_ptr, invid_rows, invtab_ptr, invtab_rows,
-                              w, b, n1_w, n1_b, w_in, b_in, w_o, b_o, nf_w, nf_b, w1, b1, w2, b2)
+                              w, b, n1_w, n1_b, w_in, b_in, w_o, b_o, nf_w, nf_b, w1, b1, w2, b2, *((idx_tab,) if indexed else ()))
         if drop_p > 0:
             out._grappa_drop = (drop_p, seed2)
         return out
@@ -605,7 +613,7 @@
     def backward(ctx, dout):
         be = get_backend()
         idx_tab = None
-        if getattr(ctx, "fused_gather", False):
+        if getattr(ctx, "fused_gather", False) or getattr(ctx, "indexed", False):
             (h, a, tab, mean1, rstd1, x1_tab, qkv, att, invid_ptr, invid_rows, invtab_ptr, invtab_rows,
              w, b, n1_w, n1_b, w_in, b_in, w_o, b_o, nf_w, nf_b, w1, b1, w2, b2, idx_tab) = ctx.saved_tensors
         else:
@@ -624,7 +632,10 @@
             _linear_bwd_params(be, dz1, sv["x3"], w1, b1, None, None)
             _linear_bwd_params(be, dzo, att, w_o, b_o, None, None)
         else:
-            if idx_tab is not None:
+            row_idx = None
+            if idx_tab is not None and getattr(be, "first_layer_indexed", False) and qkv.dtype == F32:
+                row_idx = idx_tab
+            elif idx_tab is not None:
                 qkv_tok = _new((M, 3 * Fd), tab)
                 be.tuple_gather_fwd(qkv, idx_tab, s, None, qkv_tok)
                 qkv = qkv_tok
@@ -634,13 +645,20 @@
             sz = _linear_bwd_params(be, dzo, att, w_o, b_o, satt, sz)
             datt = _new((M, Fd), qkv)
             be.gemm(dzo, w_o, datt, M=M, N=Fd, K=Fd, b_kcontig=False, a_scales=sz)
-            dqkv = _new(qkv.shape, qkv)
-            be.seqattn_bwd(qkv, datt, s, T, nheads, dqkv)
+            dqkv = _new((M, 3 * Fd), qkv)
+            if row_idx is not None:
+                be.seqattn_bwd(qkv, datt, s, T, nheads, dqkv, amax=False, row_idx=row_idx)
+            else:
+                be.seqattn_bwd(qkv, datt, s, T, nheads, dqkv)
         dqkv_tab, dres_tab = _new((s * N, 3 * Fd), qkv), _new((s * N, Fd), qkv)
-        be.tuple_gather_bwd(invtab_ptr, invtab_rows, dqkv, dqkv_tab, False, False)
-        be.tuple_gather_bwd(invtab_ptr, invtab_rows, dx2, dres_tab, False, False)
+        if getattr(be, "first_layer_indexed", False) and dqkv.dtype == F32:
+            sz = be.tuple_gather_bwd(invtab_ptr, invtab_rows, dqkv, dqkv_tab, False, False, amax=None, second=(dx2, dres_tab))
+        else:
+            be.tuple_gather_bwd(invtab_ptr, invtab_rows, dqkv, dqkv_tab, False, False)
+            be.tuple_gather_bwd(invtab_ptr, invtab_rows, dx2, dres_tab, False, False)
+            sz = None
         del dqkv
-        sz = _linear_bwd_params(be, dqkv_tab, x1_tab, w_in, b_in, sx1, None)
+        sz = _linear_bwd_params(be, dqkv_tab, x1_tab, w_in, b_in, sx1, sz)
         if hasattr(be, "credit"):
             be.credit("gemm_saved", 2.0 * 2.0 * (M - s * N) * 3 * Fd * Fd)
         dx1_tab = _new(x1_tab.shape, x1_tab)
diff --git a/grappa_amd/trainer.py b/grappa_amd/trainer.py
--- a/grappa_amd/trainer.py
+++ b/grappa_amd/trainer.py
@@ -127,7 +127,7 @@
         pw = getattr(self.model, "parameter_writer", None)
         backend_cfg = tuple(getattr(be, k, None) for k in ("gemm_precision_name", "gemm_precision_bwd_name", "inference_pairs", "training_pairs", "backward_pairs",
                                                             "_tails", "plan_override", "splitk_reduce", "weight_pairs_min_rows", "pairs_min_rows",
-                                                            "fused_writer_layer", "fused_writer_layer_bwd", "group_launches", "wgrads_aside"))
+                                                            "fused_writer_layer", "fused_writer_layer_bwd", "first_layer_indexed", "group_launches", "wgrads_aside"))
         return (float(lf.gradient_weight), float(lf.energy_weight), float(lf.param_weight), float(lf.tuplewise_weight), float(lf.proper_regularisation),
                 float(lf.improper_regularisation), tuple(sorted(lf.weights.items())), tuple(sorted(lf.param_weights_by_dataset.items())),
                 tuple(o.betas), float(o.eps), float(o.weight_decay), o.max_grad_norm, bool(self.model.training), backend_cfg,
diff --git a/include/grappa_hip.h b/include/grappa_hip.h
--- a/include/grappa_hip.h
+++ b/include/grappa_hip.h
@@ -180,6 +180,15 @@
 int grappa_seqattn_fwd_pairs_f32(void* stream, int s, int T, int nheads, int dh, const float* qkv, uint16_t* pairs, int ldp, uint32_t* out_amax);
 int grappa_seqattn_bwd_amax_f32(void* stream, int s, int T, int nheads, int dh, const float* qkv, const float* dout, float* dqkv,
                                 uint32_t* dqkv_amax);
+int grappa_seqattn_fwd_idx_f32(void* stream, int s, int T, int nheads, int dh, const float* qkv_tab, const int* row_idx, float* out,
+                               uint32_t* out_amax);
+int grappa_seqattn_fwd_pairs_idx_f32(void* stream, int s, int T, int nheads, int dh, const float* qkv_tab, const int* row_idx, uint16_t* pairs,
+                                     int ldp, uint32_t* out_amax);
+int grappa_seqattn_bwd_idx_f32(void* stream, int s, int T, int nheads, int dh, const float* qkv_tab, const int* row_idx, const float* dout,
+                               float* dqkv, uint32_t* dqkv_amax);
+int grappa_tuple_gather_bwd2_f32(void* stream, int N, const int* inv_ptr, const int* inv_rows, int has_pe, int accumulate,
+                                 int W, const float* dx, int lddx, float* da, int ldda, uint32_t* da_amax,
+                                 int W2, const float* dx2, int lddx2, float* da2, int ldda2, uint32_t* da2_amax);
 
 int grappa_perm_concat_fwd_f32(void* stream, int s, int T, int F, int P, const int* h_perm, const float* x, float* z);
 int grappa_perm_concat_bwd_f32(void* stream, int s, int T, int F, int P, const int* h_perm, const float* dz, float* dx);
```

Result: faster. 7675, median of 6 (+1.4%).
